# PRBonn/OverlapNet

Measured on AMD Instinct MI355X. Metric: scan-pairs/s (64x900 range images), higher is better.
Workload: dtype f32 (scaled 3-term fp16 split on the fp16 MFMA: 22 significand bits per operand, fp32 accumulate)

## Files before the change

overlapnet_amd/csrc/c3_dense.hip:

```cpp
#include "ovn_internal.h"

typedef _Float16 f16x8 __attribute__((ext_vector_type(8)));
typedef _Float16 f16x4 __attribute__((ext_vector_type(4)));

namespace {

struct ArithF16 {
  typedef _Float16 elem;
  typedef f16x8 v8;
  typedef f16x4 v4;
  static __device__ __forceinline__ f32x4 mfma(v8 a, v8 b, f32x4 c) { return __builtin_amdgcn_mfma_f32_16x16x32_f16(a, b, c, 0, 0, 0); }
};

constexpr int G = OVN_G;
constexpr int OW = OVN_O3_HW;
constexpr int CI = OVN_C2_OUT;
constexpr int CO = OVN_C3_OUT;
constexpr int NBAND = 3;
constexpr int MAX_ROWS = 8;
constexpr int MAX_MT = (MAX_ROWS * OW + 15) / 16;
constexpr int IN_PIX_MAX = (MAX_ROWS + 2) * G;
constexpr int PLANE = IN_PIX_MAX * 8 + 8;
constexpr int NPL = CI / 8;
constexpr size_t LDS_BYTES = 2 * (size_t)NPL * PLANE * sizeof(_Float16) + 64;
constexpr int NW = 8;

__device__ __forceinline__ int band_start(int b) { return b == 0 ? 0 : (b == 1 ? 8 : 15); }
__device__ __forceinline__ int band_rows(int b) { return b == 0 ? 8 : 7; }

constexpr int MT_SPLIT = 6;
template <class A, int NWV, int MSPLIT>
__global__ __launch_bounds__(64 * NWV) void c3_dense_kernel(const float* __restrict__ o2, const typename A::elem* __restrict__ wp,
                                                           const float* __restrict__ b3, const float* __restrict__ wd,
                                                           const unsigned* __restrict__ o2max, float sw3,
                                                           float* __restrict__ partial, float* __restrict__ o3,
                                                           unsigned* __restrict__ arrived, const float* __restrict__ bd,
                                                           float* __restrict__ overlap, float* __restrict__ logit) {
  typedef typename A::elem elem_t;
  typedef typename A::v8 v8_t;
  typedef typename A::v4 v4_t;
  extern __shared__ __attribute__((aligned(16))) unsigned char smem[];
  elem_t* ih = reinterpret_cast<elem_t*>(smem);
  elem_t* il = ih + NPL * PLANE;
  float* red = reinterpret_cast<float*>(il + NPL * PLANE);

  constexpr int HALVES = NW / NWV;
  constexpr int MTW = MSPLIT == 1 ? MAX_MT : MT_SPLIT;
  const int sub = blockIdx.x % (HALVES * MSPLIT);
  const int unit = blockIdx.x / (HALVES * MSPLIT), half = sub % HALVES, mh = sub / HALVES;
  const int mt0 = MT_SPLIT * mh;
  const int pair = unit / NBAND;
  const int band = unit - pair * NBAND;
  const int r0 = band_start(band);
  const int nrows = band_rows(band);
  const int npix = nrows * OW;
  const int nmt = (npix + 15) >> 4;
  const int tid = threadIdx.x;
  const int lane = tid & 63;
  const int wave_l = tid >> 6;
  const int wave = wave_l + NWV * half;
  const int lrow = lane & 15;
  const int g = lane >> 4;

  const elem_t* wsrc = wp + ((size_t)(2 * wave) * 2) * 512 + lane * 8;
  v8_t bq[3][4];
#define C3_LOAD_B(DST, KC)                                                                  \
  {                                                                                         \
    const elem_t* q = wsrc + (size_t)(KC) * (16 * 2 * 512);                                 \
    DST[0] = *reinterpret_cast<const v8_t*>(q);                                           \
    DST[1] = *reinterpret_cast<const v8_t*>(q + 512);                                     \
    DST[2] = *reinterpret_cast<const v8_t*>(q + 1024);                                    \
    DST[3] = *reinterpret_cast<const v8_t*>(q + 1536);                                    \
  }
  C3_LOAD_B(bq[0], 0)
  C3_LOAD_B(bq[1], 1)
  const float s2 = ovn_pow2_scale_for(__uint_as_float(o2max[pair]));
  const float inv = 1.0f / (s2 * sw3);
  {
    const float* src = o2 + ((long long)pair * G + r0) * G * CI;
    const int n4 = (nrows + 2) * G * CI / 4;
    constexpr int PER_THREAD = (MAX_ROWS + 2) * G * CI / 4 / (64 * NWV);
    static_assert(PER_THREAD * 64 * NWV == (MAX_ROWS + 2) * G * CI / 4, "patch does not divide over the threads");
    f32x4 v[PER_THREAD];
#pragma unroll
    for (int k = 0; k < PER_THREAD; ++k) {
      const int i = tid + k * (64 * NWV);
      v[k] = (i < n4) ? *reinterpret_cast<const f32x4*>(src + 4 * i) : (f32x4){0.f, 0.f, 0.f, 0.f};
    }
#pragma unroll
    for (int k = 0; k < PER_THREAD; ++k) {
      const int i = tid + k * (64 * NWV);
      if (i < n4) {
        const int pix = i / (CI / 4);
        const int c = 4 * (i - pix * (CI / 4));
        v4_t h, l;
#pragma unroll
        for (int e = 0; e < 4; ++e) {
          const float x = v[k][e] * s2;
          h[e] = (elem_t)x;
          l[e] = (elem_t)(x - (float)h[e]);
        }
        const int o = (c >> 3) * PLANE + pix * 8 + (c & 7);
        *reinterpret_cast<v4_t*>(ih + o) = h;
        *reinterpret_cast<v4_t*>(il + o) = l;
      }
    }
  }

  int abase[MTW];
#pragma unroll
  for (int mt = 0; mt < MTW; ++mt) {
    int p = 16 * (mt0 + mt) + lrow;
    if (p >= npix) p = npix - 1;
    const int oy = p / OW;
    const int ox = p - oy * OW;
    abase[mt] = g * PLANE + (oy * G + ox) * 8;
  }

  f32x4 acc[MTW][2];
#pragma unroll
  for (int mt = 0; mt < MTW; ++mt) {
    acc[mt][0] = (f32x4){0.f, 0.f, 0.f, 0.f};
    acc[mt][1] = (f32x4){0.f, 0.f, 0.f, 0.f};
  }

#define C3_MFMA2(M0, M1, A0H, A0L, A1H, A1L, SRC)                                                  \
  acc[M0][0] = A::mfma(A0H, SRC[0], acc[M0][0]);          \
  acc[M0][1] = A::mfma(A0H, SRC[2], acc[M0][1]);          \
  acc[M1][0] = A::mfma(A1H, SRC[0], acc[M1][0]);          \
  acc[M1][1] = A::mfma(A1H, SRC[2], acc[M1][1]);          \
  acc[M0][0] = A::mfma(A0L, SRC[0], acc[M0][0]);          \
  acc[M0][1] = A::mfma(A0L, SRC[2], acc[M0][1]);          \
  acc[M1][0] = A::mfma(A1L, SRC[0], acc[M1][0]);          \
  acc[M1][1] = A::mfma(A1L, SRC[2], acc[M1][1]);          \
  acc[M0][0] = A::mfma(A0H, SRC[1], acc[M0][0]);          \
  acc[M0][1] = A::mfma(A0H, SRC[3], acc[M0][1]);          \
  acc[M1][0] = A::mfma(A1H, SRC[1], acc[M1][0]);          \
  acc[M1][1] = A::mfma(A1H, SRC[3], acc[M1][1]);
#define C3_READ_A(BUF, SLOT, MT)                                                            \
  fh[BUF][SLOT] = *reinterpret_cast<const v8_t*>(ih + abase[MT] + toff);                  \
  fl[BUF][SLOT] = *reinterpret_cast<const v8_t*>(il + abase[MT] + toff);
#define C3_STEP(SRC, KC)                                                                    \
  {                                                                                         \
    const int tap = (KC) >> 2;                                                              \
    const int ky = tap / 3;                                                                 \
    const int toff = (ky * G + (tap - 3 * ky)) * 8 + 4 * PLANE * ((KC) & 3);                \
    v8_t fh[2][2], fl[2][2];                                                              \
    C3_READ_A(0, 0, 0)                                                                      \
    C3_READ_A(0, 1, 1)                                                                      \
    _Pragma("unroll") for (int q = 0; q < MTW / 2; ++q) {                                \
      const int cb = q & 1, nb = cb ^ 1;                                                    \
      if (q + 1 < MTW / 2) {                                                             \
        C3_READ_A(nb, 0, 2 * q + 2)                                                         \
        C3_READ_A(nb, 1, 2 * q + 3)                                                         \
      } else if (MTW % 2 == 1 && nmt == MAX_MT) {                                                           \
        C3_READ_A(nb, 0, MTW - 1)                                                        \
      }                                                                                     \
      __builtin_amdgcn_sched_barrier(0);   \
      C3_MFMA2(2 * q, 2 * q + 1, fh[cb][0], fl[cb][0], fh[cb][1], fl[cb][1], SRC)           \
      __builtin_amdgcn_sched_barrier(0);                                                    \
    }                                                                                       \
    if (MTW % 2 == 1 && nmt == MAX_MT) {                               \
      const v8_t ah = fh[(MTW / 2) & 1][0], al = fl[(MTW / 2) & 1][0];              \
      acc[MTW - 1][0] = A::mfma(ah, SRC[0], acc[MTW - 1][0]); \
      acc[MTW - 1][1] = A::mfma(ah, SRC[2], acc[MTW - 1][1]); \
      acc[MTW - 1][0] = A::mfma(al, SRC[0], acc[MTW - 1][0]); \
      acc[MTW - 1][1] = A::mfma(al, SRC[2], acc[MTW - 1][1]); \
      acc[MTW - 1][0] = A::mfma(ah, SRC[1], acc[MTW - 1][0]); \
      acc[MTW - 1][1] = A::mfma(ah, SRC[3], acc[MTW - 1][1]); \
    }                                                                                       \
  }
  __syncthreads();
#pragma unroll 1
  for (int kc = 0; kc < 36; kc += 3) {
    C3_LOAD_B(bq[2], kc + 2)
    C3_STEP(bq[0], kc)
    if (kc + 3 < 36) C3_LOAD_B(bq[0], kc + 3)
    C3_STEP(bq[1], kc + 1)
    if (kc + 4 < 36) C3_LOAD_B(bq[1], kc + 4)
    C3_STEP(bq[2], kc + 2)
  }
#undef C3_LOAD_B
#undef C3_STEP
#undef C3_MFMA2
#undef C3_READ_A

  float s[2] = {0.f, 0.f};
#pragma unroll
  for (int nt = 0; nt < 2; ++nt) {
    const int n = 32 * wave + 16 * nt + lrow;
    const float bv = b3[n];
#pragma unroll
    for (int mt = 0; mt < MTW; ++mt) {
#pragma unroll
      for (int r = 0; r < 4; ++r) {
        const int p = 16 * (mt0 + mt) + 4 * g + r;
        if (p < npix) {
          const float v = fmaxf(fmaf(acc[mt][nt][r], inv, bv), 0.0f);
          const long long fi = (long long)(r0 * OW + p) * CO + n;
          s[(MSPLIT == 1 && mt >= MT_SPLIT) ? 1 : 0] += v * wd[fi];
          if (o3) o3[(long long)pair * OVN_DENSE_IN + fi] = v;
        }
      }
    }
  }
#pragma unroll
  for (int off = 32; off > 0; off >>= 1) {
    s[0] += __shfl_down(s[0], off, 64);
    if (MSPLIT == 1) s[1] += __shfl_down(s[1], off, 64);
  }
  if (lane == 0) {
    red[wave_l] = s[0];
    if (MSPLIT == 1) red[NW + wave_l] = s[1];
  }
  __syncthreads();
  if (tid == 0) {
    float* dst = partial + ((size_t)pair * NBAND + band) * 4;
    if (NWV == NW) {
      dst[0] = (red[0] + red[1]) + (red[2] + red[3]);
      dst[1] = (red[NW + 0] + red[NW + 1]) + (red[NW + 2] + red[NW + 3]);
      dst[2] = (red[4] + red[5]) + (red[6] + red[7]);
      dst[3] = (red[NW + 4] + red[NW + 5]) + (red[NW + 6] + red[NW + 7]);
    } else {
      dst[2 * half + mh] = (red[0] + red[1]) + (red[2] + red[3]);
    }
    if (overlap != nullptr) {
      constexpr unsigned PARTS = NBAND * HALVES * MSPLIT;
      __threadfence();
      const unsigned prev = atomicAdd(arrived + pair, 1u);
      if (prev == PARTS - 1) {
        __threadfence();
        const float* q = partial + (size_t)pair * OVN_DENSE_PARTIALS;
        float z = 0.f;
#pragma unroll
        for (int b = 0; b < NBAND; ++b) {
          const float q0 = __hip_atomic_load(q + 4 * b, __ATOMIC_RELAXED, __HIP_MEMORY_SCOPE_AGENT);
          const float q1 = __hip_atomic_load(q + 4 * b + 1, __ATOMIC_RELAXED, __HIP_MEMORY_SCOPE_AGENT);
          const float q2 = __hip_atomic_load(q + 4 * b + 2, __ATOMIC_RELAXED, __HIP_MEMORY_SCOPE_AGENT);
          const float q3 = __hip_atomic_load(q + 4 * b + 3, __ATOMIC_RELAXED, __HIP_MEMORY_SCOPE_AGENT);
          const float zb = (q0 + q1) + (q2 + q3);
          z = b == 0 ? zb : z + zb;
        }
        z += bd[0];
        if (logit) logit[pair] = z;
        overlap[pair] = 1.0f / (1.0f + expf(-z));
        __hip_atomic_store(arrived + pair, 0u, __ATOMIC_RELAXED, __HIP_MEMORY_SCOPE_AGENT);
      }
    }
  }
}

__global__ __launch_bounds__(256) void dense_finish_kernel(const float* __restrict__ partial, const float* __restrict__ bd, int n,
                                                           float* __restrict__ overlap, float* __restrict__ logit) {
  const int p = blockIdx.x * 256 + threadIdx.x;
  if (p >= n) return;
  const float* q = partial + (size_t)p * OVN_DENSE_PARTIALS;
  float z = 0.f;
#pragma unroll
  for (int b = 0; b < NBAND; ++b) {
    const float zb = (q[4 * b] + q[4 * b + 1]) + (q[4 * b + 2] + q[4 * b + 3]);
    z = b == 0 ? zb : z + zb;
  }
  z += bd[0];
  if (logit) logit[p] = z;
  overlap[p] = 1.0f / (1.0f + expf(-z));
}

}

int ovn_c3_dense_forward(const ovn_ctx* ctx, const float* o2, const unsigned* o2max, int n, float* partial, float* o3,
                         unsigned* arrived, float* overlap, float* logit, hipStream_t stream) {
  OVN_REQUIRE(o2max != nullptr, OVN_ERR_ARG, "ovn_c3_dense_forward: the per-pair maxima of o2 are required");
  OVN_REQUIRE(overlap == nullptr || arrived != nullptr, OVN_ERR_ARG, "ovn_c3_dense_forward: arrival counters missing");
  int rc;
  if (n <= 21) {
    rc = ovn_allow_dynamic_lds(reinterpret_cast<const void*>(c3_dense_kernel<ArithF16, 4, 2>), LDS_BYTES);
    if (rc) return rc;
    hipLaunchKernelGGL((c3_dense_kernel<ArithF16, 4, 2>), dim3(4 * NBAND * n), dim3(64 * 4), LDS_BYTES, stream, o2,
                       reinterpret_cast<const _Float16*>(ctx->c3.wp_h), ctx->c3.bias, ctx->wd, o2max, ctx->c3.sw_h, partial, o3, arrived,
                       ctx->bd, overlap, logit);
  } else {
    rc = ovn_allow_dynamic_lds(reinterpret_cast<const void*>(c3_dense_kernel<ArithF16, NW, 1>), LDS_BYTES);
    if (rc) return rc;
    hipLaunchKernelGGL((c3_dense_kernel<ArithF16, NW, 1>), dim3(NBAND * n), dim3(64 * NW), LDS_BYTES, stream, o2,
                       reinterpret_cast<const _Float16*>(ctx->c3.wp_h), ctx->c3.bias, ctx->wd, o2max, ctx->c3.sw_h, partial, o3,
                       (unsigned*)nullptr, ctx->bd, (float*)nullptr, (float*)nullptr);
    if (overlap != nullptr)
      hipLaunchKernelGGL(dense_finish_kernel, dim3((n + 255) / 256), dim3(256), 0, stream, partial, ctx->bd, n, overlap, logit);
  }
  OVN_HIP_CHECK(hipGetLastError());
  return OVN_OK;
}
```

overlapnet_amd/csrc/ovn_api.hip:

```cpp
#include <stdarg.h>
#include <mutex>
#include <set>
#include <utility>
#include <stdio.h>
#include <stdlib.h>
#include <string.h>

#include <algorithm>
#include "ovn_internal.h"

int ovn_allow_dynamic_lds(const void* kernel, size_t bytes) {
  static std::mutex mu;
  static std::set<std::pair<const void*, int>> done;
  int dev = 0;
  OVN_HIP_CHECK(hipGetDevice(&dev));
  std::lock_guard<std::mutex> lock(mu);
  if (done.count({kernel, dev})) return OVN_OK;
  OVN_HIP_CHECK(hipFuncSetAttribute(kernel, hipFuncAttributeMaxDynamicSharedMemorySize, (int)bytes));
  done.insert({kernel, dev});
  return OVN_OK;
}

static thread_local char g_err[1024] = "";

void ovn_set_error(const char* fmt, ...) {
  va_list ap;
  va_start(ap, fmt);
  vsnprintf(g_err, sizeof(g_err), fmt, ap);
  va_end(ap);
}

void scratch_overwritten(ovn_ctx* ctx) {
  ctx->dbg_o2 = ctx->dbg_o3 = nullptr;
  ctx->dbg_partial = nullptr;
  ctx->dbg_o2max = nullptr;
  ctx->dbg_n = 0;
  ctx->dbg_live = nullptr;
}

int ovn_ws_reserve(ovn_ctx* ctx, size_t bytes, hipStream_t stream) {
  if (bytes <= ctx->ws_bytes) return OVN_OK;
  if (ctx->ws) {
    OVN_HIP_CHECK(hipStreamSynchronize(stream));
    OVN_HIP_CHECK(hipFree(ctx->ws));
    ctx->ws = nullptr;
    ctx->ws_bytes = 0;
    scratch_overwritten(ctx);
  }
  const size_t want = bytes + bytes / 8;
  OVN_HIP_CHECK(hipMalloc(&ctx->ws, want));
  ctx->ws_bytes = want;
  return OVN_OK;
}

static int ctx_feat_w(const ovn_ctx* ctx) { return ctx->finalized ? ctx->feat_w : OVN_FEAT_W; }

struct LegScratch {
  float* buf[2] = {nullptr, nullptr};
  double *acc = nullptr, *part = nullptr;
  LegScratch() = default;
  LegScratch(OvnCarver& c, size_t buf_elems, int nbuf, size_t acc_elems, size_t part_bytes) {
    for (int i = 0; i < nbuf; ++i) buf[i] = c.take<float>(buf_elems);
    acc = c.take<double>(acc_elems);
    part = reinterpret_cast<double*>(c.take<char>(part_bytes));
  }
};

extern "C" {

int ovn_abi_version(void) { return OVN_ABI_VERSION; }

const char* ovn_last_error(void) { return g_err; }

int ovn_create(int device_id, int in_h, int in_w, int in_c, ovn_ctx** out) {
  OVN_REQUIRE(out != nullptr, OVN_ERR_ARG, "ovn_create: out is NULL");
  OVN_REQUIRE(in_h > 0 && in_w > 0 && in_c > 0, OVN_ERR_ARG, "ovn_create: bad input shape %dx%dx%d", in_h, in_w, in_c);
  int ndev = 0;
  OVN_HIP_CHECK(hipGetDeviceCount(&ndev));
  OVN_REQUIRE(device_id >= 0 && device_id < ndev, OVN_ERR_ARG, "ovn_create: device %d not present (%d devices)", device_id, ndev);
  OVN_ON_DEVICE(device_id);
  hipDeviceProp_t prop;
  OVN_HIP_CHECK(hipGetDeviceProperties(&prop, device_id));
  OVN_REQUIRE(strncmp(prop.gcnArchName, "gfx950", 6) == 0, OVN_ERR_STATE,
              "ovn_create: this library is built for gfx950 only, device %d is %s", device_id, prop.gcnArchName);
  ovn_ctx* c = new ovn_ctx();
  c->device = device_id;
  c->in_h = in_h;
  c->in_w = in_w;
  c->in_c = in_c;
  if (const char* e = getenv("OVN_HEAD_CHUNK")) c->head_chunk = atoll(e) > 0 ? atoll(e) : c->head_chunk;
  if (const char* e = getenv("OVN_HEAD_SUBCHUNK")) c->head_sub = atoll(e) >= 0 ? atoll(e) : c->head_sub;
  if (const char* e = getenv("OVN_HEAD_STREAMS")) c->head_streams = atoi(e) == 2 ? 2 : 1;
  if (const char* e = getenv("OVN_YAW_SIDE")) c->head_yaw_side = atoi(e) ? 1 : 0;
  int rc = ovn_spectral_prepare(c, nullptr);
  if (rc) {
    ovn_conv_release(&c->dft);
    if (c->tw64) (void)hipFree(c->tw64);
    delete c;
    return rc;
  }
  *out = c;
  return OVN_OK;
}

int ovn_destroy(ovn_ctx* ctx) {
  if (!ctx) return OVN_OK;
  if (ctx->comm) (void)ovn_comm_destroy(ctx);
  OVN_ON_DEVICE(ctx->device);
  (void)hipDeviceSynchronize();
  for (auto& l : ctx->leg) ovn_conv_release(&l);
  ovn_conv_release(&ctx->c2);
  ovn_conv_release(&ctx->c3);
  ovn_conv_release(&ctx->dft);
  if (ctx->tw64) (void)hipFree(ctx->tw64);
  if (ctx->w1p) (void)hipFree(ctx->w1p);
  if (ctx->b1) (void)hipFree(ctx->b1);
  if (ctx->wd) (void)hipFree(ctx->wd);
  if (ctx->bd) (void)hipFree(ctx->bd);
  if (ctx->w1p_h) (void)hipFree(ctx->w1p_h);
  if (ctx->w2p_h) (void)hipFree(ctx->w2p_h);
  if (ctx->w1raw) (void)hipFree(ctx->w1raw);
  if (ctx->w1sum) (void)hipFree(ctx->w1sum);
  if (ctx->w1col) (void)hipFree(ctx->w1col);
  if (ctx->wsp_h) (void)hipFree(ctx->wsp_h);
  if (ctx->w2sum) (void)hipFree(ctx->w2sum);
  if (ctx->w1p_b3) (void)hipFree(ctx->w1p_b3);
  if (ctx->w2p_b3) (void)hipFree(ctx->w2p_b3);
  if (ctx->w2raw) (void)hipFree(ctx->w2raw);
  if (ctx->w3raw) (void)hipFree(ctx->w3raw);
  if (ctx->ws) (void)hipFree(ctx->ws);
  if (ctx->norm_buf) (void)hipFree(ctx->norm_buf);
  if (ctx->actmax) (void)hipFree(ctx->actmax);
  if (ctx->c3_arrived) (void)hipFree(ctx->c3_arrived);
  if (ctx->seg_dev) (void)hipFree(ctx->seg_dev);
  if (ctx->seg_host) (void)hipHostFree(ctx->seg_host);
  if (ctx->seg_ev) (void)hipEventDestroy(ctx->seg_ev);
  if (ctx->seg_done) (void)hipEventDestroy(ctx->seg_done);
  if (ctx->aux_ready) {
    for (int i = 0; i < 2; ++i) {
      (void)hipStreamDestroy(ctx->aux[i]);
      (void)hipEventDestroy(ctx->ev_join[i]);
    }
    (void)hipEventDestroy(ctx->ev_fork);
  }
  delete ctx;
  return OVN_OK;
}

static int leg_layer_prepare(OvnConvLayer* L, const float* kernel_dev, const float* bias_dev, hipStream_t stream) {
  int rc = ovn_conv_prepare(L, kernel_dev, bias_dev, stream);
  if (rc == OVN_OK) rc = ovn_conv_prepare_f16x3(L, kernel_dev, stream);
  if (rc == OVN_OK) {
    const size_t bytes = (size_t)L->kh * L->kw * L->cin * L->cout * sizeof(float);
    hipError_t e = hipMalloc((void**)&L->wraw, bytes);
    if (e == hipSuccess) e = hipMemcpyAsync(L->wraw, kernel_dev, bytes, hipMemcpyDeviceToDevice, stream);
    if (e == hipSuccess) e = hipStreamSynchronize(stream);
    if (e != hipSuccess) {
      ovn_set_error("layer %s: keeping the raw kernel failed: %s", L->name.c_str(), hipGetErrorString(e));
      rc = OVN_ERR_HIP;
    }
  }
  if (rc) ovn_conv_release(L);
  return rc;
}

int ovn_add_leg_layer(ovn_ctx* ctx, const char* name, const float* kernel_dev, const float* bias_dev, int kh, int kw,
                      int cin, int cout, int stride_h, int stride_w, void* stream) {
  OVN_REQUIRE(ctx && name && kernel_dev && bias_dev, OVN_ERR_ARG, "ovn_add_leg_layer: NULL argument");
  OVN_REQUIRE(kh > 0 && kw > 0 && cin > 0 && cout > 0 && stride_h > 0 && stride_w > 0, OVN_ERR_ARG,
              "ovn_add_leg_layer(%s): bad geometry", name);
  OVN_REQUIRE(!ctx->finalized, OVN_ERR_STATE, "ovn_add_leg_layer(%s): context already finalized", name);
  const int expect_cin = ctx->leg.empty() ? ctx->in_c : ctx->leg.back().cout;
  OVN_REQUIRE(cin == expect_cin, OVN_ERR_ARG, "ovn_add_leg_layer(%s): cin=%d but previous layer produces %d", name, cin, expect_cin);
  OVN_ON_DEVICE(ctx->device);
  OvnConvLayer L;
  L.name = name;
  L.kh = kh;
  L.kw = kw;
  L.cin = cin;
  L.cout = cout;
  L.sh = stride_h;
  L.sw = stride_w;
  L.relu = 1;
  int rc = leg_layer_prepare(&L, kernel_dev, bias_dev, (hipStream_t)stream);
  if (rc) return rc;
  ctx->leg.push_back(L);
  return OVN_OK;
}

int ovn_set_leg_layer_weights(ovn_ctx* ctx, int layer, const float* kernel_dev, const float* bias_dev, void* stream) {
  OVN_REQUIRE(ctx && kernel_dev && bias_dev, OVN_ERR_ARG, "ovn_set_leg_layer_weights: NULL argument");
  OVN_REQUIRE(ctx->finalized, OVN_ERR_STATE, "ovn_set_leg_layer_weights: context not finalized");
  OVN_REQUIRE(layer >= 0 && layer < (int)ctx->leg.size(), OVN_ERR_ARG, "ovn_set_leg_layer_weights: no such leg layer %d", layer);
  OVN_ON_DEVICE(ctx->device);
  OvnConvLayer N = ctx->leg[layer];
  N.wp = N.bias = N.wraw = nullptr;
  N.wp_h = N.wp_h16 = nullptr;
  N.sw_h = 1.f;
  int rc = leg_layer_prepare(&N, kernel_dev, bias_dev, (hipStream_t)stream);
  if (rc) return rc;
  ovn_conv_release(&ctx->leg[layer]);
  ctx->leg[layer] = N;
  return OVN_OK;
}

int ovn_set_head_weights(ovn_ctx* ctx, const float* c1k, const float* c1b, const float* c2k, const float* c2b,
                         const float* c3k, const float* c3b, const float* dk, const float* db, void* stream_) {
  OVN_REQUIRE(ctx && c1k && c1b && c2k && c2b && c3k && c3b && dk && db, OVN_ERR_ARG, "ovn_set_head_weights: NULL argument");
  OVN_ON_DEVICE(ctx->device);
  hipStream_t stream = (hipStream_t)stream_;
  {
    ovn_conv_release(&ctx->c2);
    ovn_conv_release(&ctx->c3);
    if (ctx->w1p) (void)hipFree(ctx->w1p);
    if (ctx->b1) (void)hipFree(ctx->b1);
    if (ctx->wd) (void)hipFree(ctx->wd);
    if (ctx->bd) (void)hipFree(ctx->bd);
    if (ctx->w1p_h) (void)hipFree(ctx->w1p_h);
    if (ctx->w2p_h) (void)hipFree(ctx->w2p_h);
    if (ctx->w1raw) (void)hipFree(ctx->w1raw);
    if (ctx->w1sum) (void)hipFree(ctx->w1sum);
    if (ctx->w1col) (void)hipFree(ctx->w1col);
    if (ctx->wsp_h) (void)hipFree(ctx->wsp_h);
      if (ctx->w2sum) (void)hipFree(ctx->w2sum);
    if (ctx->w1p_b3) (void)hipFree(ctx->w1p_b3);
    if (ctx->w2p_b3) (void)hipFree(ctx->w2p_b3);
    if (ctx->w2raw) (void)hipFree(ctx->w2raw);
    if (ctx->w3raw) (void)hipFree(ctx->w3raw);
    ctx->w3raw = nullptr;
    ctx->w1p_h = ctx->w2p_h = ctx->wsp_h = ctx->w1p_b3 = ctx->w2p_b3 = nullptr;
    ctx->w1raw = ctx->w1sum = ctx->w1col = ctx->w2sum = ctx->w2raw = nullptr;
    ctx->w1p = ctx->b1 = ctx->wd = ctx->bd = nullptr;
    ctx->head_set = false;
  }
  ctx->head_g = ctx_feat_w(ctx) / ctx->head_s;
  const int hs = ctx->head_s, hg = ctx->head_g;
  OVN_REQUIRE(hg >= 3, OVN_ERR_ARG, "ovn_set_head_weights: conv1size %d leaves %d column groups, c_conv3 needs 3", hs, hg);
  const bool general = (hs != OVN_S);
  int rc = OVN_OK;
  if (!general) {
    rc = ovn_delta_prepare_w1(c1k, &ctx->w1p, stream);
    if (rc) return rc;
  } else {
    const size_t w1_bytes = (size_t)hs * OVN_FEAT_C * OVN_C1_OUT * sizeof(float);
    OVN_HIP_CHECK(hipMalloc((void**)&ctx->w1raw, w1_bytes));
    OVN_HIP_CHECK(hipMemcpyAsync(ctx->w1raw, c1k, w1_bytes, hipMemcpyDeviceToDevice, stream));
  }
  OVN_HIP_CHECK(hipMalloc((void**)&ctx->b1, OVN_C1_OUT * sizeof(float)));
  OVN_HIP_CHECK(hipMemcpyAsync(ctx->b1, c1b, OVN_C1_OUT * sizeof(float), hipMemcpyDeviceToDevice, stream));
  ctx->c2 = OvnConvLayer();
  ctx->c2.name = "c_conv2";
  ctx->c2.kh = hs;
  ctx->c2.kw = 1;
  ctx->c2.cin = OVN_C1_OUT;
  ctx->c2.cout = OVN_C2_OUT;
  ctx->c2.sh = hs;
  ctx->c2.sw = 1;
  ctx->c2.relu = 1;
  rc = ovn_conv_prepare(&ctx->c2, c2k, c2b, stream);
  if (rc) return rc;
  if (!general) {
    rc = ovn_delta_prepare_f16x3(ctx, c1k, c1b, c2k, stream);
    if (rc) return rc;
  }
  ctx->c3 = OvnConvLayer();
  ctx->c3.name = "c_conv3";
  ctx->c3.kh = 3;
  ctx->c3.kw = 3;
  ctx->c3.cin = OVN_C2_OUT;
  ctx->c3.cout = OVN_C3_OUT;
  ctx->c3.sh = 1;
  ctx->c3.sw = 1;
  ctx->c3.relu = 1;
  rc = ovn_conv_prepare(&ctx->c3, c3k, c3b, stream);
  if (rc) return rc;
  if (!general) {
    rc = ovn_conv_prepare_f16x3(&ctx->c3, c3k, stream);
    if (rc) return rc;
  }
  const size_t w3_bytes = (size_t)9 * OVN_C2_OUT * OVN_C3_OUT * sizeof(float);
  OVN_HIP_CHECK(hipMalloc((void**)&ctx->w3raw, w3_bytes));
  OVN_HIP_CHECK(hipMemcpyAsync(ctx->w3raw, c3k, w3_bytes, hipMemcpyDeviceToDevice, stream));
  if (!ctx->w2raw) {
    const size_t w2_bytes = (size_t)hs * OVN_C1_OUT * OVN_C2_OUT * sizeof(float);
    OVN_HIP_CHECK(hipMalloc((void**)&ctx->w2raw, w2_bytes));
    OVN_HIP_CHECK(hipMemcpyAsync(ctx->w2raw, c2k, w2_bytes, hipMemcpyDeviceToDevice, stream));
  }
  const size_t dense_in = (size_t)(hg - 2) * (hg - 2) * OVN_C3_OUT;
  OVN_HIP_CHECK(hipMalloc((void**)&ctx->wd, dense_in * sizeof(float)));
  OVN_HIP_CHECK(hipMalloc((void**)&ctx->bd, sizeof(float)));
  OVN_HIP_CHECK(hipMemcpyAsync(ctx->wd, dk, dense_in * sizeof(float), hipMemcpyDeviceToDevice, stream));
  OVN_HIP_CHECK(hipMemcpyAsync(ctx->bd, db, sizeof(float), hipMemcpyDeviceToDevice, stream));
  OVN_HIP_CHECK(hipStreamSynchronize(stream));
  ctx->head_set = true;
  return OVN_OK;
}

static int leg_f16x3_unserved(const ovn_ctx* ctx) {
  int h = ctx->in_h, w = ctx->in_w;
  for (size_t li = 0; li < ctx->leg.size(); ++li) {
    const auto& l = ctx->leg[li];
    if (h < l.kh || w < l.kw) return -1;
    const int oh = (h - l.kh) / l.sh + 1, ow = (w - l.kw) / l.sw + 1;
    if (li == 0 && ovn_leg_front_matches(ctx, li, h, w)) {
      const auto& l2 = ctx->leg[1];
      h = (oh - l2.kh) / l2.sh + 1;
      w = (ow - l2.kw) / l2.sw + 1;
      ++li;
      continue;
    }
    if (ovn_leg_tail_matches(ctx, li, h, w)) return -1;
    if (!ovn_conv_strip_matches(l, h, w) && (long long)oh * ow < 128) return (int)li;
    h = oh;
    w = ow;
  }
  return -1;
}

int ovn_finalize(ovn_ctx* ctx, int* feat_w) {
  OVN_REQUIRE(ctx != nullptr, OVN_ERR_ARG, "ovn_finalize: ctx is NULL");
  OVN_REQUIRE(!ctx->leg.empty(), OVN_ERR_STATE, "ovn_finalize: no leg layers registered");
  int h = ctx->in_h, w = ctx->in_w, c = ctx->in_c;
  for (const auto& l : ctx->leg) {
    OVN_REQUIRE(h >= l.kh && w >= l.kw, OVN_ERR_ARG, "ovn_finalize: layer %s does not fit its %dx%d input", l.name.c_str(), h, w);
    h = (h - l.kh) / l.sh + 1;
    w = (w - l.kw) / l.sw + 1;
    c = l.cout;
  }
  OVN_REQUIRE(h == 1 && w >= OVN_FEAT_W_MIN && w <= OVN_FEAT_W_MAX && c == OVN_FEAT_C, OVN_ERR_ARG,
              "ovn_finalize: leg produces %dx%dx%d, the heads need 1 x W x %d with %d <= W <= %d", h, w, c, OVN_FEAT_C, OVN_FEAT_W_MIN,
              OVN_FEAT_W_MAX);
  OVN_REQUIRE(!ctx->head_set || w / ctx->head_s == ctx->head_g, OVN_ERR_STATE,
              "ovn_finalize: leg width %d gives %d column groups, the head weights were registered for %d", w, w / ctx->head_s,
              ctx->head_g);
  if (ctx->leg_mode != 0) {
    const int bad = leg_f16x3_unserved(ctx);
    OVN_REQUIRE(bad < 0, OVN_ERR_ARG,
                "ovn_finalize: layer %s: fewer than 128 output positions per image in leg precision f16x3 (ovn_set_leg_precision(ctx, 0) "
                "before ovn_finalize runs this leg in fp32)", ctx->leg[bad < 0 ? 0 : bad].name.c_str());
  }
  ctx->feat_w = w;
  ctx->finalized = true;
  if (feat_w) *feat_w = w;
  return OVN_OK;
}

int ovn_leg(ovn_ctx* ctx, const float* images_dev, int64_t n, float* features_dev, void* stream_) {
  OVN_REQUIRE(ctx && ctx->finalized, OVN_ERR_STATE, "ovn_leg: context not finalized");
  OVN_REQUIRE(n >= 0, OVN_ERR_ARG, "ovn_leg: n < 0");
  if (n == 0) return OVN_OK;
  OVN_REQUIRE(images_dev && features_dev, OVN_ERR_ARG, "ovn_leg: NULL buffer");
  OVN_ON_DEVICE(ctx->device);
  hipStream_t stream = (hipStream_t)stream_;
  size_t max_act = 0;
  {
    int h = ctx->in_h, w = ctx->in_w;
    for (const auto& l : ctx->leg) {
      h = (h - l.kh) / l.sh + 1;
      w = (w - l.kw) / l.sw + 1;
      const size_t e = (size_t)h * w * l.cout;
      if (e > max_act) max_act = e;
    }
  }
  const int64_t nslices = (n + OVN_LEG_SLICE - 1) / OVN_LEG_SLICE;
  const int64_t slice = (n + nslices - 1) / nslices;
  LegScratch sc;
  int rc = ovn_ws_layout(ctx, stream, &sc, (size_t)slice * max_act, 2, (size_t)0, (size_t)0);
  if (rc) return rc;
  float* const* buf = sc.buf;
  const size_t in_elems = (size_t)ctx->in_h * ctx->in_w * ctx->in_c;
  const size_t feat_elems = (size_t)ctx->feat_w * OVN_FEAT_C;
  OVN_REQUIRE(ctx->leg.size() + 1 <= OVN_ACTMAX_SLOTS, OVN_ERR_STATE, "ovn_leg: too many leg layers");
  const size_t actmax_bytes = (size_t)OVN_ACTMAX_SLOTS * OVN_LEG_SLICE * OVN_ACTMAX_STRIDE * sizeof(unsigned);
  if (ctx->leg_mode != 0 && !ctx->actmax) OVN_HIP_CHECK(hipMalloc((void**)&ctx->actmax, actmax_bytes));
  for (int64_t s0 = 0; s0 < n; s0 += slice) {
    const int nb = (int)((n - s0 < slice) ? (n - s0) : slice);
    const float* cur = images_dev + (size_t)s0 * in_elems;
    int h = ctx->in_h, w = ctx->in_w;
    if (ctx->leg_mode != 0) {
      OVN_HIP_CHECK(hipMemsetAsync(ctx->actmax, 0, (ctx->leg.size() + 1) * (size_t)slice * OVN_ACTMAX_STRIDE * sizeof(unsigned), stream));
      const bool own = (reinterpret_cast<uintptr_t>(cur) & 15) == 0 && ovn_conv_strip_own_scale(ctx->leg[0], h, w);
      if (!own) {
        OvnProfScope ps(ctx, OVN_K_LEG, stream);
        rc = ovn_absmax_forward(cur, nb, (long long)in_elems, ctx->actmax, stream);
        if (rc) return rc;
      }
    }
    for (size_t li = 0; li < ctx->leg.size(); ++li) {
      const bool last = (li + 1 == ctx->leg.size());
      float* dst = last ? features_dev + (size_t)s0 * feat_elems : buf[li & 1];
      int oh = 0, ow = 0;
      if (ctx->leg_mode != 0 && li == 0 && (reinterpret_cast<uintptr_t>(cur) & 15) == 0 && ovn_leg_front_matches(ctx, li, h, w)) {
        OvnProfScope ps(ctx, OVN_K_LEG, stream);
        float* dst2 = buf[(li + 1) & 1];
        rc = ovn_leg_front_forward(ctx, li, cur, nb, h, w, dst2, &oh, &ow, ctx->actmax + (li + 2) * (size_t)slice * OVN_ACTMAX_STRIDE, stream);
        if (rc) return rc;
        cur = dst2;
        h = oh;
        w = ow;
        ++li;
        continue;
      }
      if (ctx->leg_mode != 0 && ovn_leg_tail_matches(ctx, li, h, w)) {
        OvnProfScope ps(ctx, OVN_K_LEG, stream);
        rc = ovn_leg_tail_forward(ctx, li, cur, nb, w, features_dev + (size_t)s0 * feat_elems, stream);
        if (rc) return rc;
        break;
      }
      {
        OvnProfScope ps(ctx, OVN_K_LEG, stream);
        rc = (ctx->leg_mode == 0) ? ovn_conv_forward(ctx->leg[li], cur, nb, h, w, dst, &oh, &ow, stream)
                                  : ovn_conv_forward_f16x3(ctx->leg[li], cur, nb, h, w, dst, &oh, &ow, ctx->actmax + li * (size_t)slice * OVN_ACTMAX_STRIDE,
                                                           last ? nullptr : ctx->actmax + (li + 1) * (size_t)slice * OVN_ACTMAX_STRIDE, stream);
      }
      if (rc) return rc;
      cur = dst;
      h = oh;
      w = ow;
    }
  }
  return OVN_OK;
}

struct LegGeom {
  std::vector<int> h, w;
  std::vector<int64_t> act;
  int64_t act_total = 0, act_max = 0, params = 0;
};

static LegGeom leg_geom(const ovn_ctx* ctx) {
  LegGeom g;
  int h = ctx->in_h, w = ctx->in_w;
  for (const auto& l : ctx->leg) {
    g.h.push_back(h);
    g.w.push_back(w);
    h = (h - l.kh) / l.sh + 1;
    w = (w - l.kw) / l.sw + 1;
    g.act.push_back((int64_t)h * w * l.cout);
    g.act_total += g.act.back();
    g.act_max = std::max(g.act_max, g.act.back());
    g.params += (int64_t)l.kh * l.kw * l.cin * l.cout + l.cout;
  }
  return g;
}

int ovn_leg_layer_count(ovn_ctx* ctx, int* layers) {
  OVN_REQUIRE(ctx && layers, OVN_ERR_ARG, "ovn_leg_layer_count: NULL argument");
  *layers = (int)ctx->leg.size();
  return OVN_OK;
}

int ovn_leg_param_sizes(ovn_ctx* ctx, int64_t* sizes) {
  OVN_REQUIRE(ctx && sizes, OVN_ERR_ARG, "ovn_leg_param_sizes: NULL argument");
  for (size_t li = 0; li < ctx->leg.size(); ++li) {
    const auto& l = ctx->leg[li];
    sizes[2 * li] = (int64_t)l.kh * l.kw * l.cin * l.cout;
    sizes[2 * li + 1] = l.cout;
  }
  return OVN_OK;
}

int ovn_leg_activation_sizes(ovn_ctx* ctx, int64_t* sizes) {
  OVN_REQUIRE(ctx && sizes, OVN_ERR_ARG, "ovn_leg_activation_sizes: NULL argument");
  OVN_REQUIRE(ctx->finalized, OVN_ERR_STATE, "ovn_leg_activation_sizes: context not finalized");
  const LegGeom g = leg_geom(ctx);
  for (size_t li = 0; li < g.act.size(); ++li) sizes[li] = g.act[li];
  return OVN_OK;
}

int ovn_leg_forward_train(ovn_ctx* ctx, const float* images_dev, int64_t n, float* acts_dev, void* stream_) {
  OVN_REQUIRE(ctx && images_dev && acts_dev, OVN_ERR_ARG, "ovn_leg_forward_train: NULL argument");
  OVN_REQUIRE(n >= 1 && n < (1ll << 31), OVN_ERR_ARG, "ovn_leg_forward_train: bad n %lld", (long long)n);
  OVN_REQUIRE(ctx->finalized, OVN_ERR_STATE, "ovn_leg_forward_train: context not finalized");
  OVN_ON_DEVICE(ctx->device);
  hipStream_t stream = (hipStream_t)stream_;
  const LegGeom g = leg_geom(ctx);
  const float* cur = images_dev;
  float* dst = acts_dev;
  for (size_t li = 0; li < ctx->leg.size(); ++li) {
    OvnProfScope ps(ctx, OVN_K_LEG, stream);
    int oh = 0, ow = 0;
    int rc = ovn_conv_forward(ctx->leg[li], cur, (int)n, g.h[li], g.w[li], dst, &oh, &ow, stream);
    if (rc) return rc;
    cur = dst;
    dst += (size_t)n * g.act[li];
  }
  return OVN_OK;
}

int ovn_leg_backward(ovn_ctx* ctx, const float* images_dev, const float* acts_dev, int64_t n, const float* dfeat_dev, float* grad_dev,
                     int64_t slice_scans, void* stream_) {
  OVN_REQUIRE(ctx && images_dev && acts_dev && dfeat_dev && grad_dev, OVN_ERR_ARG, "ovn_leg_backward: NULL argument");
  OVN_REQUIRE(n >= 1 && n < (1ll << 31), OVN_ERR_ARG, "ovn_leg_backward: bad n %lld", (long long)n);
  OVN_REQUIRE(slice_scans >= 0, OVN_ERR_ARG, "ovn_leg_backward: slice_scans %lld < 0", (long long)slice_scans);
  OVN_REQUIRE(ctx->finalized, OVN_ERR_STATE, "ovn_leg_backward: context not finalized");
  OVN_ON_DEVICE(ctx->device);
  hipStream_t stream = (hipStream_t)stream_;
  const LegGeom g = leg_geom(ctx);
  const int L = (int)ctx->leg.size();
  constexpr int64_t SB = OVN_LEG_GRAD_SCAN_BLOCK;
  int64_t slice = slice_scans == 0 ? 8 * SB : std::max<int64_t>(SB, slice_scans / SB * SB);
  slice = std::min(slice, std::min<int64_t>((n + SB - 1) / SB * SB, 65535 / SB * SB));
  const int nmax = (int)std::min(slice, n);
  size_t part_bytes = 0;
  for (int li = 0; li < L; ++li) part_bytes = std::max(part_bytes, ovn_leg_grad_part_bytes(ctx->leg[li], g.h[li], g.w[li], nmax));
  LegScratch sc;
  int rc = ovn_ws_layout(ctx, stream, &sc, (size_t)nmax * g.act_max, 2, (size_t)g.params, part_bytes);
  if (rc) return rc;
  scratch_overwritten(ctx);
  float* const* buf = sc.buf;
  double *acc = sc.acc, *part = sc.part;
  OVN_HIP_CHECK(hipMemsetAsync(acc, 0, (size_t)g.params * sizeof(double), stream));
  std::vector<int64_t> act_off(L, 0), par_off(L, 0);
  for (int li = 1; li < L; ++li) {
    act_off[li] = act_off[li - 1] + g.act[li - 1];
    par_off[li] = par_off[li - 1] + (int64_t)ctx->leg[li - 1].K * ctx->leg[li - 1].cout + ctx->leg[li - 1].cout;
  }
  const size_t in_elems = (size_t)ctx->in_h * ctx->in_w * ctx->in_c;
  for (int64_t s0 = 0; s0 < n; s0 += slice) {
    const int nb = (int)std::min(slice, n - s0);
    OvnProfScope ps(ctx, OVN_K_LEG, stream);
    int cur = 0;
    rc = ovn_leg_mask_forward(dfeat_dev + (size_t)s0 * g.act[L - 1], acts_dev + (size_t)n * act_off[L - 1] + (size_t)s0 * g.act[L - 1],
                              buf[cur], (long long)nb * g.act[L - 1], stream);
    if (rc) return rc;
    for (int li = L - 1; li >= 0; --li) {
      const auto& l = ctx->leg[li];
      const float* x = li ? acts_dev + (size_t)n * act_off[li - 1] + (size_t)s0 * g.act[li - 1] : images_dev + (size_t)s0 * in_elems;
      double* ak = acc + par_off[li];
      rc = ovn_leg_layer_backward(l, x, buf[cur], nb, g.h[li], g.w[li], li ? buf[cur ^ 1] : nullptr, li ? x : nullptr, ak,
                                  ak + (int64_t)l.K * l.cout, part, stream);
      if (rc) return rc;
      cur ^= 1;
    }
  }
  return ovn_leg_grad_round(acc, grad_dev, g.params, stream);
}

int ovn_debug_conv_grad(ovn_ctx* ctx, int layer, const float* in_dev, const float* out_dev, const float* dout_dev, int nb, int h, int w,
                        float* din_dev, float* dkernel_dev, float* dbias_dev, void* stream_) {
  OVN_REQUIRE(ctx && in_dev && out_dev && dout_dev, OVN_ERR_ARG, "ovn_debug_conv_grad: NULL argument");
  OVN_REQUIRE(layer >= 0 && layer < (int)ctx->leg.size(), OVN_ERR_ARG, "ovn_debug_conv_grad: no such leg layer %d", layer);
  OVN_REQUIRE(nb >= 1 && nb <= 65535, OVN_ERR_ARG, "ovn_debug_conv_grad: bad nb %d", nb);
  const OvnConvLayer& l = ctx->leg[layer];
  OVN_REQUIRE(h >= l.kh && w >= l.kw, OVN_ERR_ARG, "ovn_debug_conv_grad: input %dx%d smaller than the kernel of %s", h, w, l.name.c_str());
  OVN_ON_DEVICE(ctx->device);
  hipStream_t stream = (hipStream_t)stream_;
  const int oh = (h - l.kh) / l.sh + 1, ow = (w - l.kw) / l.sw + 1;
  const long long out_elems = (long long)nb * oh * ow * l.cout;
  const int64_t kelems = (int64_t)l.K * l.cout;
  LegScratch sc;
  int rc = ovn_ws_layout(ctx, stream, &sc, (size_t)out_elems, 1, (size_t)(kelems + l.cout), ovn_leg_grad_part_bytes(l, h, w, nb));
  if (rc) return rc;
  scratch_overwritten(ctx);
  float* dym = sc.buf[0];
  double *acc = sc.acc, *part = sc.part;
  OVN_HIP_CHECK(hipMemsetAsync(acc, 0, (size_t)(kelems + l.cout) * sizeof(double), stream));
  OvnProfScope ps(ctx, OVN_K_LEG, stream);
  rc = ovn_leg_mask_forward(dout_dev, out_dev, dym, out_elems, stream);
  if (rc) return rc;
  rc = ovn_leg_layer_backward(l, in_dev, dym, nb, h, w, din_dev, nullptr, dkernel_dev ? acc : nullptr, dbias_dev ? acc + kelems : nullptr,
                              part, stream);
  if (rc) return rc;
  if (dkernel_dev) rc = ovn_leg_grad_round(acc, dkernel_dev, kelems, stream);
  if (rc == OVN_OK && dbias_dev) rc = ovn_leg_grad_round(acc + kelems, dbias_dev, l.cout, stream);
  return rc;
}

int ovn_corr_head(ovn_ctx* ctx, const float* feats_l, const int32_t* lidx, const float* feats_r, const int32_t* ridx,
                  int64_t n, int32_t* yaw, float* corr, void* stream) {
  OVN_REQUIRE(ctx != nullptr, OVN_ERR_ARG, "ovn_corr_head: ctx is NULL");
  OVN_REQUIRE(n >= 0 && n < (1ll << 31), OVN_ERR_ARG, "ovn_corr_head: bad n");
  if (n == 0) return OVN_OK;
  OVN_REQUIRE(feats_l && feats_r && yaw, OVN_ERR_ARG, "ovn_corr_head: NULL buffer");
  OVN_ON_DEVICE(ctx->device);
  OvnProfScope ps(ctx, OVN_K_CORR, (hipStream_t)stream);
  return ovn_corr_forward(feats_l, lidx, feats_r, ridx, (int)n, ctx_feat_w(ctx), yaw, corr, (hipStream_t)stream, ctx->corr_norm);
}

int ovn_spectrum(ovn_ctx* ctx, const float* feats_dev, int64_t n, float* spectra_dev, void* stream) {
  OVN_REQUIRE(ctx != nullptr, OVN_ERR_ARG, "ovn_spectrum: ctx is NULL");
  OVN_REQUIRE(ctx_feat_w(ctx) == OVN_FEAT_W, OVN_ERR_ARG,
              "ovn_spectrum: the spectral correlation head needs 360-column feature volumes (the leg produces %d)", ctx_feat_w(ctx));
  OVN_REQUIRE(n >= 0 && n < (1ll << 24), OVN_ERR_ARG, "ovn_spectrum: bad n");
  if (n == 0) return OVN_OK;
  OVN_REQUIRE(feats_dev && spectra_dev, OVN_ERR_ARG, "ovn_spectrum: NULL buffer");
  OVN_ON_DEVICE(ctx->device);
  OvnProfScope ps(ctx, OVN_K_SPECTRUM, (hipStream_t)stream);
  return ovn_spectrum_forward(ctx, feats_dev, (int)n, spectra_dev, (hipStream_t)stream);
}

int ovn_corr_head_spectral(ovn_ctx* ctx, const float* spec_l, const int32_t* lidx, const float* spec_r,
                           const int32_t* ridx, int64_t n, int32_t* yaw, float* corr, void* stream) {
  OVN_REQUIRE(ctx != nullptr, OVN_ERR_ARG, "ovn_corr_head_spectral: ctx is NULL");
  OVN_REQUIRE(ctx_feat_w(ctx) == OVN_FEAT_W, OVN_ERR_ARG,
              "ovn_corr_head_spectral: the spectral correlation head needs 360-column feature volumes (the leg produces %d)", ctx_feat_w(ctx));
  OVN_REQUIRE(n >= 0 && n < (1ll << 31), OVN_ERR_ARG, "ovn_corr_head_spectral: bad n");
  if (n == 0) return OVN_OK;
  OVN_REQUIRE(spec_l && spec_r && yaw, OVN_ERR_ARG, "ovn_corr_head_spectral: NULL buffer");
  OVN_ON_DEVICE(ctx->device);
  OvnProfScope ps(ctx, OVN_K_CORR_SPECTRAL, (hipStream_t)stream);
  return ovn_corr_spectral_forward(ctx, spec_l, lidx, spec_r, ridx, (int)n, yaw, corr, (hipStream_t)stream);
}

static int head_streams_ready(ovn_ctx* ctx) {
  if (ctx->aux_ready) return OVN_OK;
  for (int i = 0; i < 2; ++i) {
    OVN_HIP_CHECK(hipStreamCreateWithFlags(&ctx->aux[i], hipStreamNonBlocking));
    OVN_HIP_CHECK(hipEventCreateWithFlags(&ctx->ev_join[i], hipEventDisableTiming));
  }
  OVN_HIP_CHECK(hipEventCreateWithFlags(&ctx->ev_fork, hipEventDisableTiming));
  ctx->aux_ready = true;
  return OVN_OK;
}

struct OvnFork {
  ovn_ctx* ctx;
  hipStream_t stream;
  bool used[2] = {false, false};
  bool forked = false;
  OvnFork(ovn_ctx* c, hipStream_t s) : ctx(c), stream(s) {}
  int fork() {
    if (forked) return OVN_OK;
    int rc = head_streams_ready(ctx);
    if (rc) return rc;
    OVN_HIP_CHECK(hipEventRecord(ctx->ev_fork, stream));
    forked = true;
    return OVN_OK;
  }
  int side(int i, hipStream_t* out) {
    int rc = fork();
    if (rc) return rc;
    if (!used[i]) {
      OVN_HIP_CHECK(hipStreamWaitEvent(ctx->aux[i], ctx->ev_fork, 0));
      used[i] = true;
    }
    *out = ctx->aux[i];
    return OVN_OK;
  }
  int join() {
    int rc = OVN_OK;
    for (int i = 0; i < 2; ++i)
      if (used[i]) {
        used[i] = false;
        if (hipEventRecord(ctx->ev_join[i], ctx->aux[i]) != hipSuccess || hipStreamWaitEvent(stream, ctx->ev_join[i], 0) != hipSuccess) {
          ovn_set_error("joining the head's side stream failed");
          rc = OVN_ERR_HIP;
        }
      }
    return rc;
  }
  ~OvnFork() { (void)join(); }
};

static int delta_head_run_f32(ovn_ctx* ctx, const float* feats_l, const int32_t* lidx, const float* feats_r, const int32_t* ridx,
                              int64_t n, float* overlap, float* logit, int32_t* yaw, float* corr, int corr_mode, const float* spec_l,
                              const float* spec_r, hipStream_t stream) {
  const int fw = ctx_feat_w(ctx);
  const size_t feat_elems = (size_t)fw * OVN_FEAT_C;
  OVN_REQUIRE(corr_mode != 2 || fw == OVN_FEAT_W, OVN_ERR_ARG, "spectral correlation head at feature width %d", fw);
  const bool fusedc12 = (ctx->head_s == OVN_S);
  const size_t pb = fusedc12 ? ovn_delta_pair_bytes(ctx->head_g) : ovn_delta_generic_pair_bytes(fw, ctx->head_g);
  int64_t chunk = (int64_t)((2ull << 30) / pb);
  chunk = chunk < 1 ? 1 : (chunk > 1024 ? 1024 : chunk);
  if (ctx->head_chunk < chunk) chunk = ctx->head_chunk;
  const int64_t cmax = n < chunk ? n : chunk;
  OvnDeltaF32Scratch sc;
  OvnDeltaGenericScratch gsc;
  int rc = fusedc12 ? ovn_ws_layout(ctx, stream, &sc, cmax, ctx->head_g, ctx->head_width_split && ctx->head_mode == 1)
                    : ovn_ws_layout(ctx, stream, &gsc, cmax, fw, ctx->head_g);
  if (rc) return rc;
  scratch_overwritten(ctx);
  OvnFork fk(ctx, stream);
  if (corr_mode == 2) {
    hipStream_t ys = stream;
    if (ctx->head_yaw_side) {
      rc = fk.side(1, &ys);
      if (rc) return rc;
    }
    OvnProfScope ps(ctx, OVN_K_CORR_SPECTRAL, ys);
    rc = ovn_corr_spectral_forward(ctx, spec_l, lidx, spec_r, ridx, (int)n, yaw, corr, ys);
    if (rc) return rc;
  }
  for (int64_t p0 = 0; p0 < n; p0 += chunk) {
    const int np = (int)((n - p0 < chunk) ? (n - p0) : chunk);
    const float* fl = lidx ? feats_l : feats_l + (size_t)p0 * feat_elems;
    const int32_t* li = lidx ? lidx + p0 : nullptr;
    const int32_t* ri = ridx ? ridx + p0 : nullptr;
    if (corr_mode == 1) {
      OvnProfScope ps(ctx, OVN_K_CORR, stream);
      rc = ovn_corr_forward(fl, li, feats_r, ri, np, fw, yaw + p0, corr ? corr + (size_t)p0 * fw : nullptr, stream, ctx->corr_norm);
      if (rc) return rc;
    }
    if (fusedc12) {
      rc = ovn_delta_forward(ctx, fl, li, feats_r, ri, np, sc, overlap + p0, logit ? logit + p0 : nullptr, stream);
    } else {
      OvnProfScope ps(ctx, OVN_K_DELTA, stream);
      rc = ovn_delta_generic_forward(ctx, fl, li, feats_r, ri, np, gsc, overlap + p0, logit ? logit + p0 : nullptr, stream);
    }
    if (rc) return rc;
  }
  if (fusedc12 && n > 0 && n <= chunk) {
    ctx->dbg_o2 = sc.o2;
    ctx->dbg_o3 = sc.o3;
    ctx->dbg_n = n;
  }
  return fk.join();
}

struct HeadScratch {
  float *o2 = nullptr, *o3 = nullptr;
  char* sub = nullptr;
  size_t sub_bytes = 0;
  OvnDeltaSegScratch seg;
  HeadScratch() = default;
  HeadScratch(OvnCarver& c, int64_t cmax, bool fused, int64_t sub_pairs, int nsub, bool per_pair_right, int nseg) {
    o2 = c.take<float>((size_t)cmax * OVN_G * OVN_G * OVN_C2_OUT);
    o3 = c.take<float>((size_t)cmax * (fused ? OVN_DENSE_PARTIALS : OVN_DENSE_IN));
    sub_bytes = ovn_delta_f16x3_scratch_bytes((int)sub_pairs, per_pair_right);
    sub = c.take<char>(sub_bytes * nsub);
    if (nseg) seg = OvnDeltaSegScratch(c, nseg);
  }
  OvnDeltaSubScratch sub_chunk(int j, int np, bool per_pair_right) const {
    OvnCarver c(sub + (size_t)j * sub_bytes);
    return OvnDeltaSubScratch(c, np, per_pair_right);
  }
};

static int delta_head_run(ovn_ctx* ctx, const float* feats_l, const int32_t* lidx, const float* feats_r,
                          const int32_t* ridx, int64_t n, float* overlap, float* logit, int32_t* yaw, float* corr,
                          int corr_mode, const float* spec_l, const float* spec_r, const float* dcache_l, hipStream_t stream,
                          const OvnSegPass* seg = nullptr) {
  ctx->dbg_live = nullptr;
  const int fw = ctx_feat_w(ctx);
  if (ctx->head_s != OVN_S || fw != OVN_FEAT_W || ctx->head_mode == 0)
    return delta_head_run_f32(ctx, feats_l, lidx, feats_r, ridx, n, overlap, logit, yaw, corr, corr_mode, spec_l, spec_r, stream);
  const size_t feat_elems = (size_t)fw * OVN_FEAT_C;
  const size_t o2_elems = (size_t)OVN_G * OVN_G * OVN_C2_OUT;
  const size_t o3_elems = (size_t)OVN_DENSE_IN;
  const bool fused = (ctx->head_mode == 1);
  const int64_t chunk = ctx->head_chunk;
  const int64_t cmax = n < chunk ? n : chunk;
  int64_t sub = (!seg && ctx->head_sub > 0 && ctx->head_sub < cmax) ? ctx->head_sub : cmax;
  const int nsub_max = (int)((cmax + sub - 1) / sub);
  const int nstreams = (nsub_max > 1 && ctx->head_streams > 1) ? 2 : 1;
  HeadScratch hs;
  int rc = ovn_ws_layout(ctx, stream, &hs, cmax, fused, sub, nsub_max, ridx != nullptr, seg ? seg->nseg : 0);
  if (rc) return rc;
  if (fused && ctx->c3_arrived_n < chunk) {
    OVN_HIP_CHECK(hipStreamSynchronize(stream));
    if (ctx->c3_arrived) (void)hipFree(ctx->c3_arrived);
    ctx->c3_arrived = nullptr;
    ctx->c3_arrived_n = 0;
    OVN_HIP_CHECK(hipMalloc((void**)&ctx->c3_arrived, (size_t)chunk * sizeof(unsigned)));
    OVN_HIP_CHECK(hipMemsetAsync(ctx->c3_arrived, 0, (size_t)chunk * sizeof(unsigned), stream));
    ctx->c3_arrived_n = chunk;
  }
  float *o2 = hs.o2, *o3 = hs.o3;
  ctx->dbg_o2max = nullptr;
  ctx->dbg_o2 = o2;
  ctx->dbg_o3 = fused ? nullptr : o3;
  ctx->dbg_partial = fused ? o3 : nullptr;
  ctx->dbg_n = sub < cmax ? sub : cmax;

  OvnFork fk(ctx, stream);
  bool a2_in_yaw = false;
  if (corr_mode == 2) {
    hipStream_t ys = stream;
    if (ctx->head_yaw_side) {
      rc = fk.side(1, &ys);
      if (rc) return rc;
    }
    OvnProfScope ps(ctx, OVN_K_CORR_SPECTRAL, ys);
    a2_in_yaw = ridx == nullptr && n <= OVN_A2_IN_YAW_MAX_PAIRS && n <= chunk && ys == stream && nsub_max == 1;
    rc = ovn_corr_spectral_forward(ctx, spec_l, lidx, spec_r, ridx, (int)n, yaw, corr, ys, a2_in_yaw ? feats_r : nullptr,
                                   a2_in_yaw ? hs.sub_chunk(0, (int)n, false).a2raw : nullptr);
    if (rc) return rc;
  }
  for (int64_t c0 = 0; c0 < n; c0 += chunk) {
    const int64_t cn = (n - c0 < chunk) ? (n - c0) : chunk;
    if (corr_mode == 1) {
      OvnProfScope ps(ctx, OVN_K_CORR, stream);
      rc = ovn_corr_forward(lidx ? feats_l : feats_l + (size_t)c0 * feat_elems, lidx ? lidx + c0 : nullptr, feats_r,
                            ridx ? ridx + c0 : nullptr, (int)cn, fw, yaw + c0, corr ? corr + (size_t)c0 * fw : nullptr, stream,
                            ctx->corr_norm);
      if (rc) return rc;
    }
    int j = 0;
    for (int64_t q0 = 0; q0 < cn; q0 += sub, ++j) {
      const int64_t p0 = c0 + q0;
      const int np = (int)((cn - q0 < sub) ? (cn - q0) : sub);
      hipStream_t st = stream;
      if (nstreams == 2 && (j & 1)) {
        rc = fk.side(0, &st);
        if (rc) return rc;
      }
      const float* fl = lidx ? feats_l : feats_l + (size_t)p0 * feat_elems;
      const int32_t* li = lidx ? lidx + p0 : nullptr;
      const int32_t* ri = ridx ? ridx + p0 : nullptr;
      float* o2s = o2 + (size_t)q0 * o2_elems;
      const OvnDeltaSubScratch ds = hs.sub_chunk(j, np, ridx != nullptr);
      if (fused) {
        unsigned* o2max = ds.o2max;
        float* part = o3 + (size_t)q0 * OVN_DENSE_PARTIALS;
        OvnSegPass sp{};
        if (seg) {
          sp = *seg;
          sp.pseg += p0;
          sp.state = hs.seg;
        }
        rc = ovn_delta_c12_f16x3_forward(ctx, fl, li, feats_r, ri, np, ds, o2s, st, (int)(p0 & 0x3fffffff),
                                          dcache_l ? (lidx ? dcache_l : dcache_l + (size_t)p0 * OVN_DELTA_CACHE_ELEMS) : nullptr, a2_in_yaw,
                                          seg ? &sp : nullptr);
        if (rc) return rc;
        if (p0 == 0) ctx->dbg_o2max = o2max;
        {
          OvnProfScope ps(ctx, OVN_K_C3, st);
          rc = ovn_c3_dense_forward(ctx, o2s, o2max, np, part, nullptr, ctx->c3_arrived + q0, overlap + p0, logit ? logit + p0 : nullptr, st);
        }
      } else {
        float* o3s = o3 + (size_t)q0 * o3_elems;
        rc = ovn_delta_c12_bf16x3_forward(ctx, fl, li, feats_r, ri, np, ds, o2s, st, (int)(p0 & 0x3fffffff),
                                          a2_in_yaw);
        if (rc) return rc;
        int oh = 0, ow = 0;
        {
          OvnProfScope ps(ctx, OVN_K_C3, st);
          rc = ovn_conv_forward(ctx->c3, o2s, np, OVN_G, OVN_G, o3s, &oh, &ow, st);
        }
        if (rc) return rc;
        OvnProfScope ps(ctx, OVN_K_DENSE, st);
        rc = ovn_dense_sigmoid_forward(ctx, o3s, np, OVN_DENSE_IN, overlap + p0, logit ? logit + p0 : nullptr, st);
      }
      if (rc) return rc;
    }
  }
  return fk.join();
}

int ovn_heads(ovn_ctx* ctx, const float* feats_l, const int32_t* lidx, const float* feats_r, const int32_t* ridx,
              int64_t n, float* overlap, int32_t* yaw, float* logit, float* corr, void* stream_) {
  OVN_REQUIRE(ctx && ctx->head_set, OVN_ERR_STATE, "ovn_heads: head weights not set");
  OVN_REQUIRE(n >= 0 && n < (1ll << 31), OVN_ERR_ARG, "ovn_heads: bad n");
  if (n == 0) return OVN_OK;
  OVN_REQUIRE(feats_l && feats_r && overlap && yaw, OVN_ERR_ARG, "ovn_heads: NULL buffer");
  OVN_ON_DEVICE(ctx->device);
  return delta_head_run(ctx, feats_l, lidx, feats_r, ridx, n, overlap, logit, yaw, corr, 1, nullptr, nullptr, nullptr, (hipStream_t)stream_);
}

int ovn_heads_spectral(ovn_ctx* ctx, const float* feats_l, const float* spec_l, const float* dcache_l, const int32_t* lidx,
                       const float* feats_r, const float* spec_r, const int32_t* ridx, int64_t n, float* overlap, int32_t* yaw,
                       float* logit, float* corr, void* stream_) {
  OVN_REQUIRE(ctx && ctx->head_set, OVN_ERR_STATE, "ovn_heads_spectral: head weights not set");
  OVN_REQUIRE(ctx_feat_w(ctx) == OVN_FEAT_W, OVN_ERR_ARG,
              "ovn_heads_spectral: the spectral correlation head needs 360-column feature volumes (the leg produces %d)", ctx_feat_w(ctx));
  OVN_REQUIRE(n >= 0 && n < (1ll << 31), OVN_ERR_ARG, "ovn_heads_spectral: bad n");
  if (n == 0) return OVN_OK;
  OVN_REQUIRE(feats_l && feats_r && spec_l && spec_r && overlap && yaw, OVN_ERR_ARG, "ovn_heads_spectral: NULL buffer");
  OVN_ON_DEVICE(ctx->device);
  return delta_head_run(ctx, feats_l, lidx, feats_r, ridx, n, overlap, logit, yaw, corr, 2, spec_l, spec_r,
                        ctx->head_mode == 1 ? dcache_l : nullptr, (hipStream_t)stream_);
}

int ovn_delta_head(ovn_ctx* ctx, const float* feats_l, const int32_t* lidx, const float* feats_r, const int32_t* ridx,
                   int64_t n, float* overlap, float* logit, void* stream_) {
  OVN_REQUIRE(ctx && ctx->head_set, OVN_ERR_STATE, "ovn_delta_head: head weights not set");
  OVN_REQUIRE(n >= 0 && n < (1ll << 31), OVN_ERR_ARG, "ovn_delta_head: bad n");
  if (n == 0) return OVN_OK;
  OVN_REQUIRE(feats_l && feats_r && overlap, OVN_ERR_ARG, "ovn_delta_head: NULL buffer");
  OVN_ON_DEVICE(ctx->device);
  return delta_head_run(ctx, feats_l, lidx, feats_r, ridx, n, overlap, logit, nullptr, nullptr, 0, nullptr, nullptr, nullptr, (hipStream_t)stream_);
}

int ovn_head_param_sizes(ovn_ctx* ctx, int64_t* sizes8) {
  OVN_REQUIRE(ctx && sizes8, OVN_ERR_ARG, "ovn_head_param_sizes: NULL argument");
  ovn_head_param_sizes_of(ctx->head_s, ctx_feat_w(ctx), sizes8);
  return OVN_OK;
}

int ovn_delta_head_grad(ovn_ctx* ctx, const float* feats_l, const int32_t* lidx, const float* feats_r, const int32_t* ridx, int64_t n,
                        const float* target, int loss, float scale, float* grad, float* loss_dev, float* overlap, float* o2, float* o3,
                        void* stream_) {
  OVN_REQUIRE(ctx && feats_l && feats_r && target && grad && loss_dev, OVN_ERR_ARG, "ovn_delta_head_grad: NULL argument");
  OVN_REQUIRE(n >= 1 && n < (1ll << 31), OVN_ERR_ARG, "ovn_delta_head_grad: bad n %lld", (long long)n);
  OVN_REQUIRE(loss == 0 || loss == 1, OVN_ERR_ARG, "ovn_delta_head_grad: loss %d (0 = sigmoid loss, 1 = squared error)", loss);
  OVN_REQUIRE(isfinite(scale), OVN_ERR_ARG, "ovn_delta_head_grad: scale is not finite");
  OVN_REQUIRE(ctx->head_set, OVN_ERR_STATE, "ovn_delta_head_grad: head weights not set");
  OVN_ON_DEVICE(ctx->device);
  return ovn_delta_head_grad_run(ctx, ctx_feat_w(ctx), feats_l, lidx, feats_r, ridx, n, target, loss, scale, grad, loss_dev, overlap, o2,
                                 o3, (hipStream_t)stream_);
}

int ovn_heads_feature_grad(ovn_ctx* ctx, const float* feats_l, const int32_t* lidx, const float* feats_r, const int32_t* ridx, int64_t n,
                           const float* target, const int32_t* yaw_bin, int loss, float overlap_scale, float yaw_scale,
                           float min_overlap_for_angle, float* dfeat_l, float* dfeat_r, float* head_grad, float* loss_dev, float* overlap,
                           float* corr, void* stream_) {
  OVN_REQUIRE(ctx && feats_l && feats_r && target && dfeat_l && dfeat_r && loss_dev, OVN_ERR_ARG, "ovn_heads_feature_grad: NULL argument");
  OVN_REQUIRE(n >= 1 && n < (1ll << 31), OVN_ERR_ARG, "ovn_heads_feature_grad: bad n %lld", (long long)n);
  OVN_REQUIRE(loss == 0 || loss == 1, OVN_ERR_ARG, "ovn_heads_feature_grad: loss %d (0 = sigmoid loss, 1 = squared error)", loss);
  OVN_REQUIRE(isfinite(overlap_scale) && isfinite(yaw_scale) && isfinite(min_overlap_for_angle), OVN_ERR_ARG,
              "ovn_heads_feature_grad: a scale or the threshold is not finite");
  OVN_REQUIRE(ctx->head_set, OVN_ERR_STATE, "ovn_heads_feature_grad: head weights not set");
  const bool yaw_on = yaw_bin != nullptr && yaw_scale != 0.f;
  OVN_REQUIRE(!yaw_on || ctx->corr_norm == 0, OVN_ERR_STATE,
              "ovn_heads_feature_grad: the yaw loss is differentiated for correlation normalisation 'none' only (mode %d is set)",
              ctx->corr_norm);
  OVN_ON_DEVICE(ctx->device);
  hipStream_t stream = (hipStream_t)stream_;
  const int fw = ctx_feat_w(ctx);
  const size_t bytes = (size_t)n * fw * OVN_FEAT_C * sizeof(float);
  OVN_HIP_CHECK(hipMemsetAsync(dfeat_l, 0, bytes, stream));
  OVN_HIP_CHECK(hipMemsetAsync(dfeat_r, 0, bytes, stream));
  OVN_HIP_CHECK(hipMemsetAsync(loss_dev, 0, 2 * sizeof(float), stream));
  int rc = OVN_OK;
  if (overlap_scale != 0.f) {
    rc = ovn_delta_head_grad_run(ctx, fw, feats_l, lidx, feats_r, ridx, n, target, loss, overlap_scale, head_grad, loss_dev, overlap, nullptr,
                                 nullptr, stream, dfeat_l, dfeat_r);
  } else {
    if (head_grad) {
      int64_t sz[8], total = 0;
      ovn_head_param_sizes_of(ctx->head_s, fw, sz);
      for (int t = 0; t < 8; ++t) total += sz[t];
      OVN_HIP_CHECK(hipMemsetAsync(head_grad, 0, (size_t)total * sizeof(float), stream));
    }
    if (overlap)
      rc = ovn_delta_head_grad_run(ctx, fw, feats_l, lidx, feats_r, ridx, n, target, loss, 0.f, nullptr, nullptr, overlap, nullptr, nullptr,
                                   stream, nullptr, nullptr, true);
  }
  if (rc) return rc;
  if (yaw_on || corr)
    rc = ovn_yaw_grad_run(ctx, fw, feats_l, lidx, feats_r, ridx, n, target, yaw_on ? yaw_bin : nullptr, yaw_scale, min_overlap_for_angle,
                          dfeat_l, dfeat_r, loss_dev + 1, corr, stream);
  return rc;
}

int ovn_delta_cache(ovn_ctx* ctx, const float* feats_dev, int64_t n, float* cache_dev, void* stream) {
  OVN_REQUIRE(ctx && ctx->head_set, OVN_ERR_STATE, "ovn_delta_cache: head weights not set");
  OVN_REQUIRE(ctx_feat_w(ctx) == OVN_FEAT_W, OVN_ERR_ARG,
              "ovn_delta_cache: Delta cache rows exist for 360-column feature volumes only (the leg produces %d)", ctx_feat_w(ctx));
  OVN_REQUIRE(n >= 0 && n < (1ll << 24), OVN_ERR_ARG, "ovn_delta_cache: bad n");
  if (n == 0) return OVN_OK;
  OVN_REQUIRE(feats_dev && cache_dev, OVN_ERR_ARG, "ovn_delta_cache: NULL buffer");
  OVN_REQUIRE((reinterpret_cast<uintptr_t>(cache_dev) & 15) == 0, OVN_ERR_ARG, "ovn_delta_cache: cache_dev must be 16-byte aligned");
  OVN_REQUIRE(ctx->head_s == OVN_S, OVN_ERR_STATE, "ovn_delta_cache: only the default head geometry (conv1size 15) has a Delta cache");
  OVN_ON_DEVICE(ctx->device);
  OvnProfScope ps(ctx, OVN_K_DELTA_PREP, (hipStream_t)stream);
  return ovn_delta_cache_forward(ctx, feats_dev, (int)n, cache_dev, (hipStream_t)stream);
}

int ovn_set_head_geometry(ovn_ctx* ctx, int conv1size) {
  OVN_REQUIRE(ctx != nullptr, OVN_ERR_ARG, "ovn_set_head_geometry: ctx is NULL");
  OVN_REQUIRE(!ctx->head_set, OVN_ERR_STATE, "ovn_set_head_geometry: call it before ovn_set_head_weights");
  const int fw = ctx_feat_w(ctx);
  OVN_REQUIRE(conv1size >= 1 && fw / conv1size >= 3, OVN_ERR_ARG,
              "ovn_set_head_geometry: conv1size %d leaves fewer than 3 x 3 groups of the %d columns for c_conv3", conv1size, fw);
  ctx->head_s = conv1size;
  ctx->head_g = fw / conv1size;
  return OVN_OK;
}

int ovn_set_head_pipeline(ovn_ctx* ctx, int64_t chunk_pairs, int64_t sub_chunk_pairs, int streams, int yaw_on_side_stream) {
  OVN_REQUIRE(ctx != nullptr, OVN_ERR_ARG, "ovn_set_head_pipeline: ctx is NULL");
  OVN_REQUIRE(chunk_pairs >= 1 && chunk_pairs <= (1 << 20), OVN_ERR_ARG, "ovn_set_head_pipeline: chunk_pairs %lld", (long long)chunk_pairs);
  OVN_REQUIRE(sub_chunk_pairs >= 0, OVN_ERR_ARG, "ovn_set_head_pipeline: sub_chunk_pairs %lld", (long long)sub_chunk_pairs);
  OVN_REQUIRE(streams == 1 || streams == 2, OVN_ERR_ARG, "ovn_set_head_pipeline: streams %d (1 or 2)", streams);
  ctx->head_chunk = chunk_pairs;
  ctx->head_sub = sub_chunk_pairs;
  ctx->head_streams = streams;
  ctx->head_yaw_side = yaw_on_side_stream ? 1 : 0;
  return OVN_OK;
}

int ovn_get_head_pipeline(ovn_ctx* ctx, int64_t* chunk_pairs, int64_t* sub_chunk_pairs, int* streams, int* yaw_on_side_stream) {
  OVN_REQUIRE(ctx != nullptr, OVN_ERR_ARG, "ovn_get_head_pipeline: ctx is NULL");
  if (chunk_pairs) *chunk_pairs = ctx->head_chunk;
  if (sub_chunk_pairs) *sub_chunk_pairs = ctx->head_sub;
  if (streams) *streams = ctx->head_streams;
  if (yaw_on_side_stream) *yaw_on_side_stream = ctx->head_yaw_side;
  return OVN_OK;
}

int ovn_best_match(ovn_ctx* ctx, const float* overlap, const int32_t* yaw, const int32_t* ids, int64_t n, float threshold,
                   int64_t index_offset, int32_t* out, void* stream) {
  OVN_REQUIRE(ctx != nullptr, OVN_ERR_ARG, "ovn_best_match: ctx is NULL");
  OVN_REQUIRE(n >= 0 && n < (1ll << 31), OVN_ERR_ARG, "ovn_best_match: bad n");
  OVN_REQUIRE(index_offset >= 0 && index_offset + n < (1ll << 31), OVN_ERR_ARG, "ovn_best_match: bad index_offset");
  OVN_REQUIRE(out != nullptr && (n == 0 || overlap != nullptr), OVN_ERR_ARG, "ovn_best_match: NULL buffer");
  OVN_ON_DEVICE(ctx->device);
  return ovn_best_match_forward(overlap, yaw, ids, (int)n, threshold, (int)index_offset, out, (hipStream_t)stream);
}

int ovn_top_k(ovn_ctx* ctx, const float* overlap, const int32_t* yaw, const int32_t* ids, int64_t n, int k, float threshold,
              int64_t index_offset, int32_t* out, void* stream) {
  OVN_REQUIRE(ctx != nullptr, OVN_ERR_ARG, "ovn_top_k: ctx is NULL");
  OVN_REQUIRE(k >= 1 && k <= OVN_TOP_K_MAX, OVN_ERR_ARG, "ovn_top_k: k must be in 1..OVN_TOP_K_MAX (1024)");
  OVN_REQUIRE(n >= 0 && n < (1ll << 31), OVN_ERR_ARG, "ovn_top_k: bad n");
  OVN_REQUIRE(index_offset >= 0 && index_offset + n < (1ll << 31), OVN_ERR_ARG, "ovn_top_k: bad index_offset");
  OVN_REQUIRE(out != nullptr && (n == 0 || overlap != nullptr), OVN_ERR_ARG, "ovn_top_k: NULL buffer");
  OVN_REQUIRE((reinterpret_cast<uintptr_t>(out) & 15) == 0, OVN_ERR_ARG, "ovn_top_k: out_dev is not 16-byte aligned");
  OVN_ON_DEVICE(ctx->device);
  return ovn_top_k_forward(overlap, yaw, ids, (int)n, k, threshold, (int)index_offset, out, (hipStream_t)stream);
}

int ovn_icp_register(ovn_ctx* ctx, const float* vertex, const float* normal, const float* range, int n_scans, int proj_h, int proj_w,
                     double fov_up_deg, double fov_down_deg, double max_range, const int32_t* src_idx, const int32_t* tgt_idx,
                     int64_t n_pairs, const double* init_pose, int iterations, double max_dist, double cos_min, double huber,
                     int min_inliers, double* pose, double* stats, double* system, void* stream) {
  OVN_REQUIRE(ctx != nullptr, OVN_ERR_ARG, "ovn_icp_register: ctx is NULL");
  OVN_REQUIRE(n_scans >= 0 && proj_h > 0 && proj_w > 0 && n_pairs >= 0 && n_pairs < (1ll << 31), OVN_ERR_ARG,
              "ovn_icp_register: bad sizes");
  OVN_REQUIRE((int64_t)proj_h * proj_w <= 2147483647ll, OVN_ERR_ARG, "ovn_icp_register: H*W exceeds 2^31 - 1");
  OVN_REQUIRE(iterations >= 0 && iterations <= 1000, OVN_ERR_ARG, "ovn_icp_register: iterations must be in 0..1000");
  OVN_REQUIRE(max_dist > 0.0 && cos_min > 0.0 && huber > 0.0 && max_range > 0.0, OVN_ERR_ARG,
              "ovn_icp_register: max_dist, cos_min, huber and max_range must be > 0");
  OVN_REQUIRE(max_dist < 1e18 && cos_min <= 1.0 && huber < 1e18, OVN_ERR_ARG, "ovn_icp_register: gate out of range");
  OVN_REQUIRE(min_inliers >= 0, OVN_ERR_ARG, "ovn_icp_register: min_inliers < 0");
  OVN_REQUIRE(fabs(fov_up_deg) + fabs(fov_down_deg) > 0.0, OVN_ERR_ARG, "ovn_icp_register: empty vertical field of view");
  if (n_pairs == 0) return OVN_OK;
  OVN_REQUIRE(src_idx && tgt_idx && init_pose && pose && stats, OVN_ERR_ARG, "ovn_icp_register: NULL buffer");
  OVN_REQUIRE(n_scans == 0 || (vertex && normal && range), OVN_ERR_ARG, "ovn_icp_register: NULL image buffer");
  OVN_ON_DEVICE(ctx->device);
  return ovn_icp_register_forward(vertex, normal, range, n_scans, proj_h, proj_w, fov_up_deg, fov_down_deg, max_range, src_idx,
                                  tgt_idx, (int)n_pairs, init_pose, iterations, max_dist, cos_min, huber, min_inliers, pose, stats,
                                  system, (hipStream_t)stream);
}

struct SegTable {
  int64_t* offs = nullptr;
  int32_t *qidx = nullptr, *ridx = nullptr, *pseg = nullptr;
  SegTable() = default;
  SegTable(OvnCarver& c, int64_t B, bool with_qidx, int64_t n_ridx, int64_t n_pseg) {
    offs = c.take<int64_t>((size_t)B + 1);
    qidx = with_qidx ? c.take<int32_t>((size_t)B) : nullptr;
    ridx = n_ridx ? c.take<int32_t>((size_t)n_ridx) : nullptr;
    pseg = n_pseg ? c.take<int32_t>((size_t)n_pseg) : nullptr;
  }
};
static const char* seg_offsets_error(const int64_t* offs, int64_t B, int64_t* n_out) {
  if (B < 0 || B >= (1ll << 31)) return "B outside [0, 2^31)";
  if (!offs) return "seg_offsets is NULL";
  if (offs[0] != 0) return "seg_offsets[0] != 0";
  for (int64_t b = 0; b < B; ++b)
    if (offs[b + 1] < offs[b]) return "seg_offsets decrease";
  if (offs[B] >= (1ll << 31)) return "more than 2^31 - 1 pairs";
  *n_out = offs[B];
  return nullptr;
}

static int seg_stage(ovn_ctx* ctx, const int64_t* offs, const int32_t* qidx, int64_t B, int64_t n_ridx, int64_t n_pseg,
                     hipStream_t stream, SegTable* dev) {
  const size_t staged = ovn_scratch_bytes<SegTable>(B, qidx != nullptr, (int64_t)0, (int64_t)0);
  const size_t need = ovn_scratch_bytes<SegTable>(B, qidx != nullptr, n_ridx, n_pseg);
  if (!ctx->seg_ev) {
    OVN_HIP_CHECK(hipEventCreateWithFlags(&ctx->seg_ev, hipEventDisableTiming));
    OVN_HIP_CHECK(hipEventCreateWithFlags(&ctx->seg_done, hipEventDisableTiming));
  }
  if (ctx->seg_ev_pending) {
    OVN_HIP_CHECK(hipEventSynchronize(ctx->seg_ev));
    OVN_HIP_CHECK(hipStreamWaitEvent(stream, ctx->seg_done, 0));
    ctx->seg_ev_pending = false;
  }
  if (need > ctx->seg_cap) {
    OVN_HIP_CHECK(hipStreamSynchronize(stream));
    if (ctx->seg_dev) (void)hipFree(ctx->seg_dev);
    if (ctx->seg_host) (void)hipHostFree(ctx->seg_host);
    ctx->seg_dev = ctx->seg_host = nullptr;
    ctx->seg_cap = 0;
    const size_t want = need + need / 2;
    OVN_HIP_CHECK(hipMalloc(&ctx->seg_dev, want));
    OVN_HIP_CHECK(hipHostMalloc(&ctx->seg_host, want, hipHostMallocDefault));
    ctx->seg_cap = want;
  }
  OvnCarver hc(ctx->seg_host), dc(ctx->seg_dev);
  const SegTable h(hc, B, qidx != nullptr, n_ridx, n_pseg);
  *dev = SegTable(dc, B, qidx != nullptr, n_ridx, n_pseg);
  memcpy(h.offs, offs, (size_t)(B + 1) * sizeof(int64_t));
  if (qidx) memcpy(h.qidx, qidx, (size_t)B * sizeof(int32_t));
  OVN_HIP_CHECK(hipMemcpyAsync(ctx->seg_dev, ctx->seg_host, staged, hipMemcpyHostToDevice, stream));
  OVN_HIP_CHECK(hipEventRecord(ctx->seg_ev, stream));
  ctx->seg_ev_pending = true;
  return OVN_OK;
}

static int seg_release(ovn_ctx* ctx, hipStream_t stream) {
  OVN_HIP_CHECK(hipEventRecord(ctx->seg_done, stream));
  return OVN_OK;
}

static bool misaligned(const void* p, uintptr_t a) { return (reinterpret_cast<uintptr_t>(p) & (a - 1)) != 0; }

int ovn_heads_segments(ovn_ctx* ctx, const float* feats_pool, const float* spec_pool, const float* dcache_pool,
                       const int32_t* cand_idx, const float* feats_q, const float* spec_q, const int32_t* query_idx,
                       const int64_t* seg_offsets, int64_t B, int64_t n, float* overlap, int32_t* yaw, float* logit, float* corr,
                       void* stream_) {
  OVN_REQUIRE(ctx && ctx->head_set, OVN_ERR_STATE, "ovn_heads_segments: head weights not set");
  int64_t total = 0;
  const char* bad = seg_offsets_error(seg_offsets, B, &total);
  OVN_REQUIRE(bad == nullptr, OVN_ERR_ARG, "ovn_heads_segments: %s", bad);
  OVN_REQUIRE(n == total, OVN_ERR_ARG, "ovn_heads_segments: n = %lld but seg_offsets[B] = %lld", (long long)n, (long long)total);
  OVN_REQUIRE(B == 0 || query_idx != nullptr, OVN_ERR_ARG, "ovn_heads_segments: query_idx is NULL");
  for (int64_t b = 0; b < B; ++b)
    OVN_REQUIRE(query_idx[b] >= 0, OVN_ERR_ARG, "ovn_heads_segments: query_idx[%lld] = %d < 0", (long long)b, query_idx[b]);
  if (n == 0) return OVN_OK;
  OVN_REQUIRE(feats_pool && feats_q && cand_idx && overlap && yaw, OVN_ERR_ARG, "ovn_heads_segments: NULL buffer");
  OVN_REQUIRE((spec_pool == nullptr) == (spec_q == nullptr), OVN_ERR_ARG, "ovn_heads_segments: spec_pool and spec_q go together");
  const int fw = ctx_feat_w(ctx);
  OVN_REQUIRE(spec_pool == nullptr || fw == OVN_FEAT_W, OVN_ERR_ARG,
              "ovn_heads_segments: the spectral correlation head needs 360-column feature volumes (the leg produces %d)", fw);
  OVN_REQUIRE(!misaligned(feats_pool, 4) && !misaligned(feats_q, 4) && !misaligned(cand_idx, 4) && !misaligned(overlap, 4) &&
                  !misaligned(yaw, 4) && !misaligned(logit, 4) && !misaligned(corr, 4) && !misaligned(spec_pool, 4) &&
                  !misaligned(spec_q, 4) && !misaligned(dcache_pool, 16),
              OVN_ERR_ARG, "ovn_heads_segments: misaligned buffer (4 bytes; dcache_pool 16 bytes)");
  OVN_ON_DEVICE(ctx->device);
  hipStream_t stream = (hipStream_t)stream_;
  const bool spectral = spec_pool != nullptr;
  const int corr_mode = spectral ? 2 : 1;
  const bool segmented = ctx->head_mode == 1 && fw == OVN_FEAT_W && ctx->head_s == OVN_S && ctx->head_compact;
  SegTable tab;
  int rc = seg_stage(ctx, seg_offsets, query_idx, B, n, segmented ? n : 0, stream, &tab);
  if (rc) return rc;
  int64_t* offs_dev = tab.offs;
  int32_t *qidx_dev = tab.qidx, *ridx = tab.ridx, *pseg = tab.pseg;
  {
    OvnProfScope ps(ctx, OVN_K_DELTA_PREP, stream);
    rc = ovn_segment_ridx_forward(offs_dev, qidx_dev, (int)B, (int)n, ridx, pseg, stream);
    if (rc) return rc;
  }
  if (!segmented) {
    rc = delta_head_run(ctx, feats_pool, cand_idx, feats_q, ridx, n, overlap, logit, yaw, corr, corr_mode, spec_pool, spec_q, nullptr, stream);
    return rc ? rc : seg_release(ctx, stream);
  }
  const float* dc = spectral ? dcache_pool : nullptr;
  const int64_t* o = seg_offsets;
  auto seg_of = [&](int64_t p) { return (int64_t)(std::upper_bound(o, o + B + 1, p) - o) - 1; };
  for (int64_t p0 = 0; p0 < n;) {
    const int64_t b0 = seg_of(p0);
    int64_t p1 = std::min(n, p0 + ctx->head_chunk);
    if (seg_of(p1 - 1) - b0 + 1 > OVN_SEG_PASS_MAX) p1 = o[b0 + OVN_SEG_PASS_MAX];
    const int64_t np = p1 - p0;
    OvnSegPass sp{pseg + p0, qidx_dev, offs_dev, (int)b0, (int)(seg_of(p1 - 1) - b0 + 1), {}};
    rc = delta_head_run(ctx, feats_pool, cand_idx + p0, feats_q, ridx + p0, np, overlap + p0, logit ? logit + p0 : nullptr, yaw + p0,
                        corr ? corr + (size_t)p0 * fw : nullptr, corr_mode, spec_pool, spec_q, dc, stream, &sp);
    if (rc) return rc;
    p0 = p1;
  }
  return seg_release(ctx, stream);
}

int ovn_top_k_segments(ovn_ctx* ctx, const float* overlap, const int32_t* yaw, const int32_t* ids, const int64_t* seg_offsets,
                       int64_t B, int k, float threshold, int32_t* out, void* stream) {
  OVN_REQUIRE(ctx != nullptr, OVN_ERR_ARG, "ovn_top_k_segments: ctx is NULL");
  OVN_REQUIRE(k >= 1 && k <= OVN_TOP_K_MAX, OVN_ERR_ARG, "ovn_top_k_segments: k must be in 1..OVN_TOP_K_MAX (1024)");
  int64_t n = 0;
  const char* bad = seg_offsets_error(seg_offsets, B, &n);
  OVN_REQUIRE(bad == nullptr, OVN_ERR_ARG, "ovn_top_k_segments: %s", bad);
  if (B == 0) return OVN_OK;
  OVN_REQUIRE(out != nullptr && (n == 0 || overlap != nullptr), OVN_ERR_ARG, "ovn_top_k_segments: NULL buffer");
  OVN_REQUIRE(!misaligned(out, 16), OVN_ERR_ARG, "ovn_top_k_segments: out_dev is not 16-byte aligned");
  OVN_REQUIRE(!misaligned(overlap, 4) && !misaligned(yaw, 4) && !misaligned(ids, 4), OVN_ERR_ARG,
              "ovn_top_k_segments: misaligned buffer");
  OVN_ON_DEVICE(ctx->device);
  SegTable tab;
  int rc = seg_stage(ctx, seg_offsets, nullptr, B, 0, 0, (hipStream_t)stream, &tab);
  if (rc) return rc;
  rc = ovn_top_k_segments_forward(overlap, yaw, ids, tab.offs, (int)B, k, threshold, out, (hipStream_t)stream);
  return rc ? rc : seg_release(ctx, (hipStream_t)stream);
}

int ovn_project(ovn_ctx* ctx, const float* points_dev, const int64_t* offsets_dev, int n_scans,
                int64_t max_points_per_scan, int proj_h, int proj_w, double fov_up_deg, double fov_down_deg,
                double max_range, float* range_dev, float* vertex_dev, float* intensity_dev, int32_t* idx_dev,
                float* normal_dev, float* stacked_dev, int use_depth, int use_normals, int use_intensity, void* stream) {
  OVN_REQUIRE(ctx != nullptr, OVN_ERR_ARG, "ovn_project: ctx is NULL");
  OVN_REQUIRE(n_scans == 0 || (points_dev || max_points_per_scan == 0), OVN_ERR_ARG, "ovn_project: points is NULL");
  OVN_REQUIRE(n_scans == 0 || offsets_dev, OVN_ERR_ARG, "ovn_project: offsets is NULL");
  OVN_ON_DEVICE(ctx->device);
  OvnProfScope ps(ctx, OVN_K_PROJ, (hipStream_t)stream);
  return ovn_project_forward(ctx, points_dev, offsets_dev, n_scans, max_points_per_scan, proj_h, proj_w, fov_up_deg,
                             fov_down_deg, max_range, range_dev, vertex_dev, intensity_dev, idx_dev, normal_dev,
                             stacked_dev, use_depth, use_normals, use_intensity, (hipStream_t)stream);
}

int ovn_project_semantic(ovn_ctx* ctx, const float* points_dev, const int64_t* offsets_dev, int n_scans,
                         int64_t max_points_per_scan, int proj_h, int proj_w, double fov_up_deg, double fov_down_deg,
                         double max_range, const float* probs_dev, int n_classes, float* range_dev, float* vertex_dev,
                         float* intensity_dev, int32_t* idx_dev, float* normal_dev, float* semantic_dev, int32_t* sem_idx_dev,
                         float* stacked_dev, int use_depth, int use_normals, int use_semantic, int use_intensity, void* stream) {
  OVN_REQUIRE(n_classes >= 1 && n_classes <= OVN_SEMANTIC_CLASSES_MAX, OVN_ERR_ARG,
              "ovn_project_semantic: n_classes %d outside 1..%d", n_classes, OVN_SEMANTIC_CLASSES_MAX);
  OVN_REQUIRE(probs_dev || !(semantic_dev || (stacked_dev && use_semantic)), OVN_ERR_ARG,
              "ovn_project_semantic: probabilities requested but probs is NULL");
  OVN_REQUIRE(ctx != nullptr, OVN_ERR_ARG, "ovn_project_semantic: ctx is NULL");
  OVN_REQUIRE(n_scans == 0 || (points_dev || max_points_per_scan == 0), OVN_ERR_ARG, "ovn_project_semantic: points is NULL");
  OVN_REQUIRE(n_scans == 0 || offsets_dev, OVN_ERR_ARG, "ovn_project_semantic: offsets is NULL");
  OVN_ON_DEVICE(ctx->device);
  OvnProfScope ps(ctx, OVN_K_PROJ, (hipStream_t)stream);
  return ovn_project_semantic_forward(ctx, points_dev, offsets_dev, n_scans, max_points_per_scan, proj_h, proj_w, fov_up_deg,
                                      fov_down_deg, max_range, probs_dev, n_classes, range_dev, vertex_dev, intensity_dev, idx_dev,
                                      normal_dev, semantic_dev, sem_idx_dev, stacked_dev, use_depth, use_normals, use_semantic,
                                      use_intensity, (hipStream_t)stream);
}

int ovn_projection_angles(ovn_ctx* ctx, const float* points_dev, int64_t n_points, int proj_h, int proj_w, double fov_up_deg,
                          double fov_down_deg, double max_range, float* yaw_dev, float* pitch_dev, int32_t* pixel_dev,
                          void* stream) {
  OVN_REQUIRE(ctx != nullptr, OVN_ERR_ARG, "ovn_projection_angles: ctx is NULL");
  OVN_REQUIRE(n_points >= 0 && proj_h > 0 && proj_w > 0, OVN_ERR_ARG, "ovn_projection_angles: bad sizes");
  if (n_points == 0) return OVN_OK;
  OVN_REQUIRE(points_dev != nullptr, OVN_ERR_ARG, "ovn_projection_angles: points is NULL");
  OVN_ON_DEVICE(ctx->device);
  return ovn_projection_angles_forward(points_dev, n_points, proj_h, proj_w, fov_up_deg, fov_down_deg, max_range, yaw_dev,
                                       pitch_dev, pixel_dev, (hipStream_t)stream, ctx->proj_trig);
}

int ovn_normals(ovn_ctx* ctx, const float* range_dev, const float* vertex_dev, int n_scans, int proj_h, int proj_w,
                float* normal_dev, void* stream) {
  OVN_REQUIRE(ctx != nullptr, OVN_ERR_ARG, "ovn_normals: ctx is NULL");
  OVN_REQUIRE(n_scans >= 0 && proj_h > 0 && proj_w > 0, OVN_ERR_ARG, "ovn_normals: bad sizes");
  if (n_scans == 0) return OVN_OK;
  OVN_REQUIRE(range_dev && vertex_dev && normal_dev, OVN_ERR_ARG, "ovn_normals: NULL buffer");
  OVN_ON_DEVICE(ctx->device);
  return ovn_normals_forward(range_dev, vertex_dev, n_scans, proj_h, proj_w, normal_dev, (hipStream_t)stream);
}

int ovn_gt_range_images(ovn_ctx* ctx, const float* points_dev, const int64_t* offsets_dev, int n_scans,
                        int64_t max_points_per_scan, const double* ref_poses_dev, const double* inv_cur_pose_dev, int proj_h,
                        int proj_w, double fov_up_deg, double fov_down_deg, double max_range, float* range_dev, void* stream) {
  OVN_REQUIRE(ctx != nullptr, OVN_ERR_ARG, "ovn_gt_range_images: ctx is NULL");
  OVN_REQUIRE(n_scans >= 0 && proj_h > 0 && proj_w > 0 && max_points_per_scan >= 0, OVN_ERR_ARG, "ovn_gt_range_images: bad sizes");
  if (n_scans == 0) return OVN_OK;
  OVN_REQUIRE(offsets_dev && range_dev && (points_dev || max_points_per_scan == 0), OVN_ERR_ARG, "ovn_gt_range_images: NULL buffer");
  OVN_REQUIRE(n_scans <= 65535, OVN_ERR_ARG, "ovn_gt_range_images: at most 65535 scans per call");
  OVN_ON_DEVICE(ctx->device);
  return ovn_gt_range_forward(points_dev, offsets_dev, n_scans, max_points_per_scan, ref_poses_dev, inv_cur_pose_dev, proj_h,
                              proj_w, fov_up_deg, fov_down_deg, max_range, range_dev, (hipStream_t)stream);
}

int ovn_gt_overlap_counts(ovn_ctx* ctx, const float* ref_ranges_dev, const float* cur_range_dev, int n_scans, int proj_h,
                          int proj_w, int32_t* counts_dev, void* stream) {
  OVN_REQUIRE(ctx != nullptr, OVN_ERR_ARG, "ovn_gt_overlap_counts: ctx is NULL");
  OVN_REQUIRE(n_scans >= 0 && proj_h > 0 && proj_w > 0, OVN_ERR_ARG, "ovn_gt_overlap_counts: bad sizes");
  OVN_REQUIRE(cur_range_dev && counts_dev && (ref_ranges_dev || n_scans == 0), OVN_ERR_ARG, "ovn_gt_overlap_counts: NULL buffer");
  OVN_ON_DEVICE(ctx->device);
  return ovn_gt_count_forward(ref_ranges_dev, cur_range_dev, n_scans, proj_h * proj_w, counts_dev, (hipStream_t)stream);
}

int ovn_gt_pair_counts(ovn_ctx* ctx, const float* points_dev, const int64_t* offsets_dev, int n_scans, const double* poses_dev,
                       const double* inv_poses_dev, const float* cur_ranges_dev, const int32_t* frame_idx_dev, int n_frames,
                       const int32_t* ref_idx_dev, int n_refs, int proj_h, int proj_w, double fov_up_deg, double fov_down_deg,
                       double max_range, int32_t* counts_dev, void* stream) {
  OVN_REQUIRE(ctx != nullptr, OVN_ERR_ARG, "ovn_gt_pair_counts: ctx is NULL");
  OVN_REQUIRE(n_scans >= 0 && n_frames >= 0 && n_refs >= 0 && proj_h > 0 && proj_w > 0, OVN_ERR_ARG,
              "ovn_gt_pair_counts: bad sizes");
  OVN_REQUIRE((long long)proj_h * proj_w <= 262144, OVN_ERR_ARG,
              "ovn_gt_pair_counts: %d x %d pixels need %lld bytes of LDS for the two bit planes, 65536 at the most (H*W <= 262144)",
              proj_h, proj_w, 8ll * (((long long)proj_h * proj_w + 31) / 32));
  OVN_REQUIRE((long long)n_frames * n_refs <= 2147483647ll, OVN_ERR_ARG,
              "ovn_gt_pair_counts: %d frames x %d references exceed the grid (2^31 - 1 pairs per call)", n_frames, n_refs);
  if (n_frames == 0 || n_refs == 0) return OVN_OK;
  OVN_REQUIRE(counts_dev != nullptr, OVN_ERR_ARG, "ovn_gt_pair_counts: counts is NULL");
  OVN_REQUIRE(n_scans > 0 && offsets_dev && poses_dev && inv_poses_dev && cur_ranges_dev, OVN_ERR_ARG,
              "ovn_gt_pair_counts: NULL buffer");
  OVN_REQUIRE((frame_idx_dev || n_frames <= n_scans) && (ref_idx_dev || n_refs <= n_scans), OVN_ERR_ARG,
              "ovn_gt_pair_counts: without an index list at most n_scans (%d) frames / references", n_scans);
  int frame_fastest = 1;
  if (const char* e = getenv("OVN_GT_PAIR_ORDER")) frame_fastest = e[0] == 'r' ? 0 : 1;
  OVN_ON_DEVICE(ctx->device);
  return ovn_gt_pair_forward(points_dev, offsets_dev, n_scans, poses_dev, inv_poses_dev, cur_ranges_dev, frame_idx_dev, n_frames,
                             ref_idx_dev, n_refs, proj_h, proj_w, fov_up_deg, fov_down_deg, max_range, frame_fastest, counts_dev,
                             (hipStream_t)stream);
}

int ovn_set_head_precision(ovn_ctx* ctx, int mode) {
  OVN_REQUIRE(ctx != nullptr, OVN_ERR_ARG, "ovn_set_head_precision: ctx is NULL");
  OVN_REQUIRE(mode >= 0 && mode <= 2, OVN_ERR_ARG, "ovn_set_head_precision: mode %d (0 = fp32 MFMA, 1 = f16x3 MFMA, 2 = bf16x3 MFMA)", mode);
  ctx->head_mode = mode;
  return OVN_OK;
}

int ovn_set_head_width_split(ovn_ctx* ctx, int on) {
  OVN_REQUIRE(ctx != nullptr, OVN_ERR_ARG, "ovn_set_head_width_split: ctx is NULL");
  OVN_REQUIRE(on == 0 || on == 1, OVN_ERR_ARG, "ovn_set_head_width_split: %d (0 = exact fp32 at widths other than 360, 1 = f16x3 there)", on);
  ctx->head_width_split = on;
  return OVN_OK;
}

int ovn_get_head_width_split(ovn_ctx* ctx, int* on) {
  OVN_REQUIRE(ctx != nullptr && on != nullptr, OVN_ERR_ARG, "ovn_get_head_width_split: NULL argument");
  *on = ctx->head_width_split;
  return OVN_OK;
}

int ovn_set_corr_normalization(ovn_ctx* ctx, int mode) {
  OVN_REQUIRE(ctx != nullptr, OVN_ERR_ARG, "ovn_set_corr_normalization: ctx is NULL");
  OVN_REQUIRE(mode >= 0 && mode <= 3, OVN_ERR_ARG,
              "ovn_set_corr_normalization: mode %d (0 = none, 1 = euclidean, 2 = scaling, 3 = standardization)", mode);
  ctx->corr_norm = mode;
  return OVN_OK;
}

int ovn_get_corr_normalization(ovn_ctx* ctx, int* mode) {
  OVN_REQUIRE(ctx != nullptr && mode != nullptr, OVN_ERR_ARG, "ovn_get_corr_normalization: NULL argument");
  *mode = ctx->corr_norm;
  return OVN_OK;
}

int ovn_set_head_compaction(ovn_ctx* ctx, int on) {
  OVN_REQUIRE(ctx != nullptr, OVN_ERR_ARG, "ovn_set_head_compaction: ctx is NULL");
  OVN_REQUIRE(on == 0 || on == 1, OVN_ERR_ARG, "ovn_set_head_compaction: %d (0 = walk all 128 channels, 1 = drop the query's dead channels)", on);
  ctx->head_compact = on;
  return OVN_OK;
}

int ovn_set_projection_trig(ovn_ctx* ctx, int mode) {
  OVN_REQUIRE(ctx != nullptr, OVN_ERR_ARG, "ovn_set_projection_trig: ctx is NULL");
  OVN_REQUIRE(mode == 0 || mode == 1, OVN_ERR_ARG, "ovn_set_projection_trig: mode %d (0 = NumPy / SVML float32, 1 = correctly rounded)", mode);
  ctx->proj_trig = mode;
  return OVN_OK;
}

int ovn_set_leg_precision(ovn_ctx* ctx, int mode) {
  OVN_REQUIRE(ctx != nullptr, OVN_ERR_ARG, "ovn_set_leg_precision: ctx is NULL");
  OVN_REQUIRE(mode == 0 || mode == 1, OVN_ERR_ARG, "ovn_set_leg_precision: mode %d (0 = fp32 MFMA, 1 = f16x3 MFMA)", mode);
  if (mode != 0 && ctx->finalized) {
    const int bad = leg_f16x3_unserved(ctx);
    OVN_REQUIRE(bad < 0, OVN_ERR_ARG, "ovn_set_leg_precision: layer %s: fewer than 128 output positions per image in leg precision f16x3",
                ctx->leg[bad < 0 ? 0 : bad].name.c_str());
  }
  ctx->leg_mode = mode;
  return OVN_OK;
}

int ovn_profile_begin(ovn_ctx* ctx) {
  OVN_REQUIRE(ctx != nullptr, OVN_ERR_ARG, "ovn_profile_begin: ctx is NULL");
  for (auto& r : ctx->prof_recs) {
    (void)hipEventDestroy(r.a);
    (void)hipEventDestroy(r.b);
  }
  ctx->prof_recs.clear();
  ctx->prof = true;
  return OVN_OK;
}

int ovn_profile_end(ovn_ctx* ctx, double* ms_by_kind, int64_t* launches_by_kind) {
  OVN_REQUIRE(ctx && ms_by_kind && launches_by_kind, OVN_ERR_ARG, "ovn_profile_end: NULL argument");
  OVN_ON_DEVICE(ctx->device);
  ctx->prof = false;
  for (int k = 0; k < OVN_K_COUNT; ++k) {
    ms_by_kind[k] = 0.0;
    launches_by_kind[k] = 0;
  }
  int rc = OVN_OK;
  for (auto& r : ctx->prof_recs) {
    float ms = 0.f;
    hipError_t e = hipEventSynchronize(r.b);
    if (e == hipSuccess) e = hipEventElapsedTime(&ms, r.a, r.b);
    if (e != hipSuccess) {
      ovn_set_error("ovn_profile_end: %s", hipGetErrorString(e));
      rc = OVN_ERR_HIP;
    } else {
      ms_by_kind[r.kind] += ms;
      launches_by_kind[r.kind] += 1;
    }
    (void)hipEventDestroy(r.a);
    (void)hipEventDestroy(r.b);
  }
  ctx->prof_recs.clear();
  return rc;
}

int ovn_debug_conv(ovn_ctx* ctx, int layer, const float* in_dev, int nb, int h, int w, float* out_dev, void* stream) {
  OVN_REQUIRE(ctx && layer >= 0 && layer < (int)ctx->leg.size(), OVN_ERR_ARG, "ovn_debug_conv: no such leg layer");
  OVN_REQUIRE(in_dev && out_dev && nb >= 0, OVN_ERR_ARG, "ovn_debug_conv: bad buffers");
  OVN_ON_DEVICE(ctx->device);
  int oh = 0, ow = 0;
  if (ctx->leg_mode == 0) return ovn_conv_forward(ctx->leg[layer], in_dev, nb, h, w, out_dev, &oh, &ow, (hipStream_t)stream);
  OVN_REQUIRE(nb <= OVN_LEG_SLICE, OVN_ERR_ARG, "ovn_debug_conv: at most %d images per call", OVN_LEG_SLICE);
  if (!ctx->actmax) OVN_HIP_CHECK(hipMalloc((void**)&ctx->actmax, (size_t)OVN_ACTMAX_SLOTS * OVN_LEG_SLICE * OVN_ACTMAX_STRIDE * sizeof(unsigned)));
  OVN_HIP_CHECK(hipMemsetAsync(ctx->actmax, 0, 2 * (size_t)OVN_LEG_SLICE * OVN_ACTMAX_STRIDE * sizeof(unsigned), (hipStream_t)stream));
  int rc = ovn_absmax_forward(in_dev, nb, (long long)h * w * ctx->leg[layer].cin, ctx->actmax, (hipStream_t)stream);
  if (rc) return rc;
  return ovn_conv_forward_f16x3(ctx->leg[layer], in_dev, nb, h, w, out_dev, &oh, &ow, ctx->actmax, ctx->actmax + (size_t)OVN_LEG_SLICE * OVN_ACTMAX_STRIDE,
                                (hipStream_t)stream);
}

int ovn_debug_head_activations(ovn_ctx* ctx, int64_t n, float* o2_dev, float* o3_dev, void* stream) {
  OVN_REQUIRE(ctx && ctx->dbg_o2 && n >= 0 && n <= ctx->dbg_n, OVN_ERR_STATE,
              "ovn_debug_head_activations: call right after ovn_heads with n <= its (first-chunk) pair count");
  OVN_ON_DEVICE(ctx->device);
  const size_t g = (size_t)ctx->head_g;
  if (o2_dev)
    OVN_HIP_CHECK(hipMemcpyAsync(o2_dev, ctx->dbg_o2, (size_t)n * g * g * OVN_C2_OUT * sizeof(float),
                                 hipMemcpyDeviceToDevice, (hipStream_t)stream));
  if (o3_dev && ctx->dbg_o3)
    OVN_HIP_CHECK(hipMemcpyAsync(o3_dev, ctx->dbg_o3, (size_t)n * (g - 2) * (g - 2) * OVN_C3_OUT * sizeof(float),
                                 hipMemcpyDeviceToDevice, (hipStream_t)stream));
  else if (o3_dev)
    return ovn_c3_dense_forward(ctx, ctx->dbg_o2, ctx->dbg_o2max, (int)n, ctx->dbg_partial, o3_dev, nullptr, nullptr, nullptr, (hipStream_t)stream);
  return OVN_OK;
}

int ovn_head_walk_stats(ovn_ctx* ctx, int32_t* out16_host, void* stream) {
  OVN_REQUIRE(ctx && out16_host, OVN_ERR_ARG, "ovn_head_walk_stats: NULL argument");
  OVN_ON_DEVICE(ctx->device);
  return ovn_delta_walk_stats(ctx, out16_host, (hipStream_t)stream);
}

int64_t ovn_workspace_bytes(ovn_ctx* ctx) { return ctx ? (int64_t)ctx->ws_bytes : 0; }

int ovn_selftest(ovn_ctx* ctx) {
  OVN_REQUIRE(ctx != nullptr, OVN_ERR_ARG, "ovn_selftest: ctx is NULL");
  OVN_ON_DEVICE(ctx->device);
  return ovn_mfma_selftest(nullptr);
}

}
```

overlapnet_amd/csrc/ovn_internal.h:

```cpp
#pragma once

#include <hip/hip_runtime.h>
#include <math.h>
#include <stdint.h>

#include <string>
#include <vector>

#include "../../include/ovn_hip.h"
#include "ovn_scratch.h"

typedef float f32x4 __attribute__((ext_vector_type(4)));

void ovn_set_error(const char* fmt, ...);

#define OVN_HIP_CHECK(expr)                                                                   \
  do {                                                                                        \
    hipError_t _e = (expr);                                                                   \
    if (_e != hipSuccess) {                                                                   \
      ovn_set_error("%s failed: %s (%s:%d)", #expr, hipGetErrorString(_e), __FILE__, __LINE__); \
      return OVN_ERR_HIP;                                                                     \
    }                                                                                         \
  } while (0)

#define OVN_REQUIRE(cond, code, ...)   \
  do {                                 \
    if (!(cond)) {                     \
      ovn_set_error(__VA_ARGS__);      \
      return (code);                   \
    }                                  \
  } while (0)

struct OvnDeviceGuard {
  int prev = -1;
  bool ok = false;
  explicit OvnDeviceGuard(int dev) {
    int cur = -1;
    if (hipGetDevice(&cur) != hipSuccess) return;
    if (cur == dev) {
      ok = true;
      return;
    }
    ok = (hipSetDevice(dev) == hipSuccess);
    if (ok) prev = cur;
  }
  ~OvnDeviceGuard() {
    if (prev >= 0) (void)hipSetDevice(prev);
  }
  OvnDeviceGuard(const OvnDeviceGuard&) = delete;
  OvnDeviceGuard& operator=(const OvnDeviceGuard&) = delete;
};
#define OVN_ON_DEVICE(dev)                                                             \
  OvnDeviceGuard ovn_device_guard_(dev);                                               \
  OVN_REQUIRE(ovn_device_guard_.ok, OVN_ERR_HIP, "cannot select HIP device %d", (int)(dev))

constexpr int OVN_FEAT_W = 360;
constexpr int OVN_FEAT_C = 128;
constexpr int OVN_FEAT_ELEMS = OVN_FEAT_W * OVN_FEAT_C;
constexpr int OVN_S = 15;
constexpr int OVN_G = OVN_FEAT_W / OVN_S;
constexpr int OVN_C1_OUT = 64;
constexpr int OVN_C2_OUT = 128;
constexpr int OVN_C3_OUT = 256;
constexpr int OVN_O3_HW = OVN_G - 2;
constexpr int OVN_DENSE_IN = OVN_O3_HW * OVN_O3_HW * OVN_C3_OUT;
constexpr int OVN_A2_IN_YAW_MAX_PAIRS = 64;
constexpr int OVN_DENSE_PARTIALS = 12;
constexpr int OVN_ACTMAX_SLOTS = 32;
constexpr int OVN_LEG_SLICE = 1024;
constexpr int OVN_ACTMAX_STRIDE = 32;
constexpr int OVN_SPEC_W = 368;
constexpr int OVN_SPEC_ELEMS = OVN_FEAT_C * OVN_SPEC_W;
static_assert(OVN_DELTA_CACHE_ELEMS >= OVN_FEAT_ELEMS + 24 * 128 + 4, "include/ovn_hip.h: OVN_DELTA_CACHE_ELEMS");

__host__ __device__ inline float ovn_pow2_scale_for(float m) {
  if (!(m > 0.0f) || !(m < 3.0e38f)) return 1.0f;
  int e = 0;
  (void)frexpf(m, &e);
  int k = 14 - e;
  k = k > 100 ? 100 : (k < -100 ? -100 : k);
  return ldexpf(1.0f, k);
}

#ifdef __HIPCC__
__device__ __forceinline__ void ovn_fold_absmax_wg(float vmax, unsigned* word, float* red) {
#pragma unroll
  for (int off = 32; off > 0; off >>= 1) vmax = fmaxf(vmax, __shfl_down(vmax, off, 64));
  const int nw = (blockDim.x + 63) >> 6;
  if ((threadIdx.x & 63) == 0) red[threadIdx.x >> 6] = vmax;
  __syncthreads();
  if (threadIdx.x == 0) {
    float m = red[0];
    for (int w = 1; w < nw; ++w) m = fmaxf(m, red[w]);
    const unsigned bits = __float_as_uint(m);
    if (m > 0.f && bits > __hip_atomic_load(word, __ATOMIC_RELAXED, __HIP_MEMORY_SCOPE_AGENT)) atomicMax(word, bits);
  }
}

template <int NWAVES>
__device__ __forceinline__ float ovn_wg_max_all(float m, float* red) {
#pragma unroll
  for (int off = 32; off > 0; off >>= 1) m = fmaxf(m, __shfl_down(m, off, 64));
  if ((threadIdx.x & 63) == 0) red[threadIdx.x >> 6] = m;
  __syncthreads();
  m = red[0];
#pragma unroll
  for (int w = 1; w < NWAVES; ++w) m = fmaxf(m, red[w]);
  return m;
}

typedef _Float16 f16x8 __attribute__((ext_vector_type(8)));
typedef _Float16 f16x4 __attribute__((ext_vector_type(4)));
typedef _Float16 f16x2 __attribute__((ext_vector_type(2)));

__device__ __forceinline__ void ovn_split_f16(float d0, float d1, float s, float one, f16x2& hi, f16x2& lo) {
  const float x0 = d0 * s, x1 = d1 * s;
  hi = __builtin_bit_cast(f16x2, __builtin_amdgcn_cvt_pkrtz(x0, x1));
  lo[0] = (_Float16)__builtin_fmaf(x0, one, -(float)hi[0]);
  lo[1] = (_Float16)__builtin_fmaf(x1, one, -(float)hi[1]);
}
__device__ __forceinline__ void ovn_split_f16(f32x4 d, float s, float one, f16x4& hi, f16x4& lo) {
#pragma unroll
  for (int e = 0; e < 4; e += 2) {
    f16x2 h, l;
    ovn_split_f16(d[e], d[e + 1], s, one, h, l);
    hi[e] = h[0];
    hi[e + 1] = h[1];
    lo[e] = l[0];
    lo[e + 1] = l[1];
  }
}
#endif

constexpr int OVN_NORM_BLK = 24;
constexpr int OVN_NORM_NB = OVN_FEAT_W / OVN_NORM_BLK;
static_assert(OVN_NORM_NB * OVN_NORM_BLK == OVN_FEAT_W, "15 whole blocks tile the 360 columns (the spectral kernels' LDS)");
constexpr int OVN_NORM_NB_MAX = (OVN_FEAT_W_MAX + OVN_NORM_BLK - 1) / OVN_NORM_BLK;

template <int NB, int NCH>
struct OvnNormLds {
  double part[NB][NCH];
  float mn[NB][NCH], mx[NB][NCH];
  double m[NCH], s[NCH];
};

__host__ __device__ inline double ovn_corr_norm_add(int mode) { return mode == 3 ? 1e-5 : 0.0; }

#ifdef __HIPCC__
__device__ __forceinline__ float ovn_corr_norm_apply(float x, double m, double a, double s) {
  return (float)((((double)x - m) + a) * s);
}

__device__ __forceinline__ void ovn_norm_block_stats(const float* __restrict__ p, int n, double& sm, float& lo, float& hi) {
#pragma unroll 8
  for (int i = 0; i < n; ++i) {
    const float v = p[(size_t)i * OVN_FEAT_C];
    sm += (double)v;
    lo = fminf(lo, v);
    hi = fmaxf(hi, v);
  }
}
__device__ __forceinline__ double ovn_norm_block_sumsq(const float* __restrict__ p, int n, double m, double a) {
  double q = 0.0;
#pragma unroll 8
  for (int i = 0; i < n; ++i) {
    const double y = ((double)p[(size_t)i * OVN_FEAT_C] - m) + a;
    q = __builtin_fma(y, y, q);
  }
  return q;
}

template <int NB, int NCH>
__device__ void ovn_corr_norm_affine(const float* __restrict__ X, int W, int mode, OvnNormLds<NB, NCH>& L) {
  const int tid = threadIdx.x, nt = blockDim.x;
  const int nfull = W / OVN_NORM_BLK, tail = W - nfull * OVN_NORM_BLK, nb = nfull + (tail ? 1 : 0);
  for (int t = tid; t < nb * NCH; t += nt) {
    const int c = t % NCH, b = t / NCH;
    const float* p = X + (size_t)(b * OVN_NORM_BLK) * OVN_FEAT_C + c;
    double sm = 0.0;
    float lo = INFINITY, hi = -INFINITY;
    if (b < nfull) ovn_norm_block_stats(p, OVN_NORM_BLK, sm, lo, hi);
    else ovn_norm_block_stats(p, tail, sm, lo, hi);
    L.part[b][c] = sm;
    L.mn[b][c] = lo;
    L.mx[b][c] = hi;
  }
  __syncthreads();
  if (tid < NCH) {
    double sm = 0.0;
    float lo = INFINITY, hi = -INFINITY;
    for (int b = 0; b < nb; ++b) {
      sm += L.part[b][tid];
      lo = fminf(lo, L.mn[b][tid]);
      hi = fmaxf(hi, L.mx[b][tid]);
    }
    if (mode == 2) {
      L.m[tid] = (double)lo;
      L.s[tid] = 1.0 / (((double)hi - (double)lo) + 1e-6);
    } else {
      L.m[tid] = (mode == 3) ? sm / (double)W : 0.0;
      L.s[tid] = 0.0;
    }
  }
  __syncthreads();
  if (mode == 2) return;
  const double a = ovn_corr_norm_add(mode);
  for (int t = tid; t < nb * NCH; t += nt) {
    const int c = t % NCH, b = t / NCH;
    const float* p = X + (size_t)(b * OVN_NORM_BLK) * OVN_FEAT_C + c;
    L.part[b][c] = ovn_norm_block_sumsq(p, b < nfull ? OVN_NORM_BLK : tail, L.m[c], a);
  }
  __syncthreads();
  if (tid < NCH) {
    double q = 0.0;
    for (int b = 0; b < nb; ++b) q += L.part[b][tid];
    L.s[tid] = 1.0 / sqrt(q > 1e-12 ? q : 1e-12);
  }
  __syncthreads();
}
#endif

struct OvnHeadScales {
  float sw1 = 1.f, sw2 = 1.f;
  float sws = 1.f;
  float w1_colsum = 0.f;
  float b1_absmax = 0.f;
};

int ovn_allow_dynamic_lds(const void* kernel, size_t bytes);

struct OvnConvLayer {
  std::string name;
  int kh = 0, kw = 0, cin = 0, cout = 0, sh = 1, sw = 1;
  int relu = 1;
  int out_cols = 0;
  int K = 0;
  int nkc = 0;
  float* wp = nullptr;
  float* bias = nullptr;
  void* wp_h = nullptr;
  float sw_h = 1.f;
  void* wp_h16 = nullptr;
  float* wraw = nullptr;
};

struct ovn_ctx {
  int device = 0;
  int in_h = 0, in_w = 0, in_c = 0;
  std::vector<OvnConvLayer> leg;
  bool finalized = false;
  int feat_w = 0;
  bool head_set = false;
  int head_s = OVN_S;
  int head_g = OVN_G;
  float* w1p = nullptr;
  float* b1 = nullptr;
  OvnConvLayer c2;
  OvnConvLayer c3;
  void* w1p_h = nullptr;
  void* w2p_h = nullptr;
  float* w1raw = nullptr;
  float* w1sum = nullptr;
  float* w1col = nullptr;
  void* wsp_h = nullptr;
  float* w2sum = nullptr;
  void* w1p_b3 = nullptr;
  void* w2p_b3 = nullptr;
  float* w2raw = nullptr;
  float* w3raw = nullptr;
  OvnHeadScales hs;
  int leg_mode = 1;
  int head_compact = 1;
  int proj_trig = 0;
  unsigned* actmax = nullptr;
  int head_mode = 1;
  int head_width_split = 0;
  float* wd = nullptr;
  float* bd = nullptr;
  OvnConvLayer dft;
  double* tw64 = nullptr;
  int corr_norm = 0;
  float* norm_buf = nullptr;
  int64_t norm_buf_n = 0;
  void* comm = nullptr;
  int comm_rank = 0, comm_world = 1;
  int64_t head_chunk = 1024;
  int64_t head_sub = 0;
  int head_streams = 1;
  int head_yaw_side = 0;
  bool aux_ready = false;
  hipStream_t aux[2] = {nullptr, nullptr};
  hipEvent_t ev_fork = nullptr, ev_join[2] = {nullptr, nullptr};
  void* ws = nullptr;
  size_t ws_bytes = 0;
  bool prof = false;
  struct ProfRec {
    hipEvent_t a, b;
    int kind;
  };
  std::vector<ProfRec> prof_recs;
  const float* dbg_o2 = nullptr;
  const float* dbg_o3 = nullptr;
  float* dbg_partial = nullptr;
  const unsigned* dbg_o2max = nullptr;
  int64_t dbg_n = 0;
  unsigned* c3_arrived = nullptr;
  int64_t c3_arrived_n = 0;
  const unsigned* dbg_live = nullptr;
  void* seg_host = nullptr;
  void* seg_dev = nullptr;
  size_t seg_cap = 0;
  hipEvent_t seg_ev = nullptr;
  hipEvent_t seg_done = nullptr;
  bool seg_ev_pending = false;
};

enum { OVN_K_LEG = 0, OVN_K_CORR = 1, OVN_K_DELTA = 2, OVN_K_C3 = 3, OVN_K_DENSE = 4, OVN_K_PROJ = 5, OVN_K_SPECTRUM = 6,
       OVN_K_CORR_SPECTRAL = 7, OVN_K_DELTA_PREP = 8, OVN_K_DELTA_C2 = 9, OVN_K_COUNT = 10 };

struct OvnProfScope {
  ovn_ctx* ctx;
  hipStream_t stream;
  hipEvent_t a = nullptr, b = nullptr;
  int kind;
  OvnProfScope(ovn_ctx* c, int k, hipStream_t s) : ctx(c), stream(s), kind(k) {
    if (ctx->prof && hipEventCreate(&a) == hipSuccess && hipEventCreate(&b) == hipSuccess) (void)hipEventRecord(a, stream);
  }
  ~OvnProfScope() {
    if (ctx->prof && a && b) {
      (void)hipEventRecord(b, stream);
      ctx->prof_recs.push_back({a, b, kind});
    }
  }
};

int ovn_ws_reserve(ovn_ctx* ctx, size_t bytes, hipStream_t stream);
void scratch_overwritten(ovn_ctx* ctx);
template <class L, class... A>
int ovn_ws_layout(ovn_ctx* ctx, hipStream_t stream, L* out, const A&... a) {
  int rc = ovn_ws_reserve(ctx, ovn_scratch_bytes<L>(a...), stream);
  if (rc) return rc;
  OvnCarver c(ctx->ws);
  *out = L(c, a...);
  return OVN_OK;
}

int ovn_conv_prepare(OvnConvLayer* L, const float* kernel_dev, const float* bias_dev, hipStream_t stream);
void ovn_conv_release(OvnConvLayer* L);
int ovn_conv_forward(const OvnConvLayer& L, const float* in, int nb, int h, int w, float* out, int* oh,
                     int* ow, hipStream_t stream);

int ovn_conv_prepare_f16x3(OvnConvLayer* L, const float* kernel_dev, hipStream_t stream);
int ovn_conv_forward_f16x3(const OvnConvLayer& L, const float* in, int nb, int h, int w, float* out, int* oh, int* ow,
                           const unsigned* in_max, unsigned* out_max, hipStream_t stream);
int ovn_absmax_forward(const float* x, int n_scans, long long per_scan, unsigned* out_max, hipStream_t stream);

int ovn_delta_prepare_w1(const float* c1_kernel_dev, float** w1p_out, hipStream_t stream);
struct OvnDeltaF32Scratch {
  float *o2 = nullptr, *o3 = nullptr;
  void* scales = nullptr;
  OvnDeltaF32Scratch() = default;
  OvnDeltaF32Scratch(OvnCarver& c, int64_t n, int G, bool split);
};
size_t ovn_delta_pair_bytes(int G);
int ovn_delta_forward(ovn_ctx* ctx, const float* feats_l, const int32_t* lidx, const float* feats_r, const int32_t* ridx, int n,
                      const OvnDeltaF32Scratch& scratch, float* overlap, float* logit, hipStream_t stream);
int ovn_dense_sigmoid_forward(const ovn_ctx* ctx, const float* o3, int n, long long dense_in, float* overlap, float* logit,
                              hipStream_t stream);

int ovn_delta_prepare_f16x3(ovn_ctx* ctx, const float* c1_kernel_dev, const float* c1_bias_dev, const float* c2_kernel_dev,
                            hipStream_t stream);
struct OvnDeltaSubScratch {
  f32x4* scales = nullptr;
  unsigned *o2max = nullptr, *pl = nullptr, *pr = nullptr;
  float *lin = nullptr, *a2raw = nullptr, *o1raw = nullptr;
  void* desc = nullptr;
  unsigned *qblock = nullptr, *live = nullptr;
  _Float16* w1c = nullptr;
  OvnDeltaSubScratch() = default;
  OvnDeltaSubScratch(OvnCarver& c, int n, bool per_pair_right);
};
struct OvnDeltaSegScratch {
  float* a2raw = nullptr;
  unsigned *qblock = nullptr, *live = nullptr;
  _Float16* w1c = nullptr;
  OvnDeltaSegScratch() = default;
  OvnDeltaSegScratch(OvnCarver& c, int nseg);
};
size_t ovn_delta_f16x3_scratch_bytes(int n, bool per_pair_right);
struct OvnSegPass {
  const int32_t* pseg;
  const int32_t* qidx;
  const int64_t* offs;
  int seg0, nseg;
  OvnDeltaSegScratch state;
};
size_t ovn_delta_f16x3_seg_bytes(int nseg);
int ovn_delta_c12_f16x3_forward(ovn_ctx* ctx, const float* feats_l, const int32_t* lidx, const float* feats_r,
                                const int32_t* ridx, int n, const OvnDeltaSubScratch& scratch, float* o2, hipStream_t stream,
                                int pair0 = 0,
                                const float* dcache_l = nullptr,
                                bool a2_done = false,
                                const struct OvnSegPass* seg = nullptr);
int ovn_delta_c12_bf16x3_forward(ovn_ctx* ctx, const float* feats_l, const int32_t* lidx, const float* feats_r, const int32_t* ridx,
                                 int n, const OvnDeltaSubScratch& scratch, float* o2, hipStream_t stream, int pair0, bool a2_done);
int ovn_delta_cache_forward(ovn_ctx* ctx, const float* feats, int n, float* cache, hipStream_t stream);
int ovn_delta_walk_stats(ovn_ctx* ctx, int32_t* out16, hipStream_t stream);

struct OvnDeltaGenericScratch {
  float *out1 = nullptr, *o2 = nullptr, *o3 = nullptr;
  OvnDeltaGenericScratch() = default;
  OvnDeltaGenericScratch(OvnCarver& c, int64_t n, int W, int G);
};
size_t ovn_delta_generic_pair_bytes(int W, int G);
int ovn_delta_generic_forward(const ovn_ctx* ctx, const float* feats_l, const int32_t* lidx, const float* feats_r,
                              const int32_t* ridx, int n, const OvnDeltaGenericScratch& scratch, float* overlap, float* logit,
                              hipStream_t stream);
int ovn_delta_generic_c1_wide(const ovn_ctx* ctx, int FW, const float* feats_l, const int32_t* lidx, const float* feats_r,
                              const int32_t* ridx, int n, float* out1, hipStream_t stream);

void ovn_head_param_sizes_of(int s, int FW, int64_t* sizes8);
int ovn_delta_head_grad_run(ovn_ctx* ctx, int FW, const float* feats_l, const int32_t* lidx, const float* feats_r, const int32_t* ridx,
                            int64_t n, const float* target, int loss, float scale, float* grad, float* loss_out, float* overlap,
                            float* o2_out, float* o3_out, hipStream_t stream,
                            float* dfeat_l = nullptr, float* dfeat_r = nullptr,
                            bool forward_only = false);

int ovn_delta_data_grad(ovn_ctx* ctx, int FW, const float* feats_l, const int32_t* lidx, const float* feats_r, const int32_t* ridx,
                        const float* dO1, int np, float* dfeat_l, float* dfeat_r, hipStream_t stream);
int ovn_yaw_grad_run(ovn_ctx* ctx, int FW, const float* feats_l, const int32_t* lidx, const float* feats_r, const int32_t* ridx,
                     int64_t n, const float* target, const int32_t* yaw_bin, float yaw_scale, float thr, float* dfeat_l, float* dfeat_r,
                     float* loss_yaw, float* corr, hipStream_t stream);

size_t ovn_leg_grad_part_bytes(const OvnConvLayer& L, int h, int w, int nb);
int ovn_leg_mask_forward(const float* dy, const float* y, float* out, long long n, hipStream_t stream);
int ovn_leg_grad_round(const double* acc, float* out, long long n, hipStream_t stream);
int ovn_leg_layer_backward(const OvnConvLayer& L, const float* x, const float* dym, int nb, int h, int w, float* dx, const float* mask,
                           double* acc_kernel, double* acc_bias, double* part, hipStream_t stream);

size_t ovn_delta_w_split_pair_bytes();
int ovn_delta_w_split_c12_forward(ovn_ctx* ctx, const float* feats_l, const int32_t* lidx, const float* feats_r, const int32_t* ridx,
                                  int n, void* scales, float* o2, hipStream_t stream);

int ovn_corr_forward(const float* feats_l, const int32_t* lidx, const float* feats_r, const int32_t* ridx, int n, int W,
                     int32_t* yaw, float* corr, hipStream_t stream, int norm_mode);

int ovn_spectral_prepare(ovn_ctx* ctx, hipStream_t stream);
int ovn_spectrum_forward(ovn_ctx* ctx, const float* feats, int n, float* spectra, hipStream_t stream);
bool ovn_conv_strip_own_scale(const OvnConvLayer& L, int h, int w);
bool ovn_conv_strip_matches(const OvnConvLayer& L, int h, int w);
int ovn_conv_strip_try(const OvnConvLayer& L, const float* in, int nb, int h, int w, float* out, const unsigned* in_max,
                       unsigned* out_max, hipStream_t stream);

bool ovn_leg_front_matches(const ovn_ctx* ctx, size_t first, int h, int w);
int ovn_leg_front_forward(const ovn_ctx* ctx, size_t first, const float* in, int nb, int h, int w, float* out, int* oh_out, int* ow_out,
                          unsigned* out_max, hipStream_t stream);

bool ovn_leg_tail_matches(const ovn_ctx* ctx, size_t first, int h, int w);
int ovn_leg_tail_forward(const ovn_ctx* ctx, size_t first, const float* in, int nb, int w, float* out, hipStream_t stream);

int ovn_c3_dense_forward(const ovn_ctx* ctx, const float* o2, const unsigned* o2max, int n, float* partial, float* o3,
                         unsigned* arrived, float* overlap, float* logit, hipStream_t stream);

int ovn_gt_range_forward(const float* points, const int64_t* offsets, int n_scans, long long max_points, const double* ref_poses,
                         const double* inv_cur_pose, int H, int W, double fov_up_deg, double fov_down_deg, double max_range,
                         float* range_out, hipStream_t stream);
int ovn_gt_count_forward(const float* ref_ranges, const float* cur_range, int n, int npix, int32_t* counts, hipStream_t stream);
int ovn_gt_pair_forward(const float* points, const int64_t* offsets, int n_scans, const double* poses, const double* inv_poses,
                        const float* cur_ranges, const int32_t* frame_idx, int n_frames, const int32_t* ref_idx, int n_refs, int H,
                        int W, double fov_up_deg, double fov_down_deg, double max_range, int frame_fastest, int32_t* counts,
                        hipStream_t stream);
int ovn_best_match_forward(const float* overlap, const int32_t* yaw, const int32_t* ids, int n, float threshold,
                           int index_offset, int32_t* out, hipStream_t stream);
int ovn_top_k_forward(const float* overlap, const int32_t* yaw, const int32_t* ids, int n, int k, float threshold,
                      int index_offset, int32_t* out, hipStream_t stream);
int ovn_top_k_segments_forward(const float* overlap, const int32_t* yaw, const int32_t* ids, const int64_t* offs_dev, int B, int k,
                               float threshold, int32_t* out, hipStream_t stream);
int ovn_segment_ridx_forward(const int64_t* offs_dev, const int32_t* qidx_dev, int B, int n, int32_t* ridx, int32_t* pseg,
                             hipStream_t stream);
int ovn_icp_register_forward(const float* vertex, const float* normal, const float* range, int n_scans, int H, int W,
                             double fov_up_deg, double fov_down_deg, double max_range, const int32_t* src_idx, const int32_t* tgt_idx,
                             int n_pairs, const double* init_pose, int iterations, double max_dist, double cos_min, double huber,
                             int min_inliers, double* pose, double* stats, double* system, hipStream_t stream);
int ovn_corr_spectral_forward(ovn_ctx* ctx, const float* spec_l, const int32_t* lidx, const float* spec_r,
                              const int32_t* ridx, int n, int32_t* yaw, float* corr, hipStream_t stream,
                              const float* a2_feats_r = nullptr, float* a2raw = nullptr);

int ovn_project_forward(ovn_ctx* ctx, const float* points, const int64_t* offsets, int n_scans,
                        int64_t max_points, int H, int W, double fov_up_deg, double fov_down_deg,
                        double max_range, float* range, float* vertex, float* intensity, int32_t* idx,
                        float* normal, float* stacked, int use_depth, int use_normals, int use_intensity,
                        hipStream_t stream);

int ovn_project_semantic_forward(ovn_ctx* ctx, const float* points, const int64_t* offsets, int n_scans, int64_t max_points, int H,
                                 int W, double fov_up_deg, double fov_down_deg, double max_range, const float* probs, int n_classes,
                                 float* range, float* vertex, float* intensity, int32_t* idx, float* normal, float* semantic,
                                 int32_t* sem_idx, float* stacked, int use_depth, int use_normals, int use_semantic, int use_intensity,
                                 hipStream_t stream);
int ovn_projection_angles_forward(const float* points, int64_t n, int H, int W, double fov_up_deg, double fov_down_deg,
                                  double max_range, float* yaw, float* pitch, int32_t* pixel, hipStream_t stream, int trig = 0);
int ovn_normals_forward(const float* range, const float* vertex, int n_scans, int H, int W, float* normal,
                        hipStream_t stream);

int ovn_mfma_selftest(hipStream_t stream);
```

Baseline: 235,700.

## Split conv3+dense into six pixel-tile bands with fragment-ordered dense weights

Replaces the three row bands of the fused conv3+Dense kernel with six bands of up to six 16-pixel M-tiles, cut in raster pixel order. It uses 4-wave workgroups tuned for two workgroups per CU, and the number of N-tiles per wave is a template parameter (1, 2 or 4) picked from the batch size. Dense weights are reordered once, at setup, into MFMA fragment order so the epilogue can read them contiguously. The change is meant to improve occupancy and load balance, and to shrink the LDS patch per workgroup. In exchange there are more partials per pair (96 instead of 12), which need a separate partial buffer and a longer finishing reduction, and some input halo is reloaded across bands.

```diff
diff --git a/overlapnet_amd/csrc/c3_bands.h b/overlapnet_amd/csrc/c3_bands.h
--- /dev/null
+++ b/overlapnet_amd/csrc/c3_bands.h
@@ -0,0 +1,45 @@
+#pragma once
+
+constexpr int C3B_G = 24;
+constexpr int C3B_OW = 22;
+constexpr int C3B_CI = 128;
+constexpr int C3B_CO = 256;
+constexpr int C3B_NPIX = C3B_OW * C3B_OW;
+constexpr int C3B_TILES = (C3B_NPIX + 15) / 16;
+constexpr int C3B_NBAND = 6;
+constexpr int C3B_MAX_MT = 6;
+constexpr int C3B_NT = C3B_CO / 16;
+
+constexpr int c3b_first_tile(int b) { return 5 * b; }
+constexpr int c3b_tiles(int b) { return b == C3B_NBAND - 1 ? C3B_TILES - c3b_first_tile(b) : 5; }
+constexpr int c3b_first_pixel(int b) { return 16 * c3b_first_tile(b); }
+constexpr int c3b_pixels(int b) { return b == C3B_NBAND - 1 ? C3B_NPIX - c3b_first_pixel(b) : 16 * c3b_tiles(b); }
+constexpr int c3b_raster(int p) { return (p / C3B_OW) * C3B_G + p % C3B_OW; }
+constexpr int C3B_TAP_MAX = 2 * C3B_G + 2;
+constexpr int c3b_origin(int b) { return c3b_raster(c3b_first_pixel(b)); }
+constexpr int c3b_span(int b) { return c3b_raster(c3b_first_pixel(b) + c3b_pixels(b) - 1) + C3B_TAP_MAX + 1 - c3b_origin(b); }
+constexpr int c3b_max_span() {
+  int m = 0;
+  for (int b = 0; b < C3B_NBAND; ++b) m = c3b_span(b) > m ? c3b_span(b) : m;
+  return m;
+}
+constexpr int C3B_MAX_SPAN = c3b_max_span();
+
+constexpr int C3B_NPL = C3B_CI / 8;
+constexpr int C3B_PLANE = C3B_MAX_SPAN * 8 + 8;
+constexpr int C3B_LDS_BYTES = 2 * C3B_NPL * C3B_PLANE * 2;
+constexpr int C3B_PATCH_LOADS = (C3B_MAX_SPAN * C3B_CI / 4 + 255) / 256;
+
+constexpr int C3B_WDF_ELEMS = C3B_NBAND * C3B_NT * C3B_MAX_MT * 64 * 4;
+constexpr int c3b_wdf_index(int band, int nt, int mt, int lane, int r) {
+  return (((band * C3B_NT + nt) * C3B_MAX_MT + mt) * 64 + lane) * 4 + r;
+}
+constexpr int c3b_wdf_source(int band, int nt, int mt, int lane, int r) {
+  const int p = 16 * mt + 4 * (lane >> 4) + r;
+  return (mt < c3b_tiles(band) && p < c3b_pixels(band)) ? (c3b_first_pixel(band) + p) * C3B_CO + 16 * nt + (lane & 15) : -1;
+}
+
+static_assert(c3b_first_tile(C3B_NBAND - 1) + c3b_tiles(C3B_NBAND - 1) == C3B_TILES && c3b_tiles(C3B_NBAND - 1) == C3B_MAX_MT, "bands");
+static_assert(c3b_origin(C3B_NBAND - 1) + c3b_span(C3B_NBAND - 1) == C3B_G * C3B_G, "the last band ends with the input");
+static_assert(C3B_PATCH_LOADS <= 18, "patch loads per thread");
+static_assert(C3B_LDS_BYTES <= 80 * 1024 && 2 * C3B_LDS_BYTES <= 160 * 1024, "two workgroups share a CU's 160 KB of LDS");
diff --git a/overlapnet_amd/csrc/c3_dense.hip b/overlapnet_amd/csrc/c3_dense.hip
--- a/overlapnet_amd/csrc/c3_dense.hip
+++ b/overlapnet_amd/csrc/c3_dense.hip
@@ -1,7 +1,5 @@
 #include "ovn_internal.h"
-
-typedef _Float16 f16x8 __attribute__((ext_vector_type(8)));
-typedef _Float16 f16x4 __attribute__((ext_vector_type(4)));
+#include "c3_bands.h"
 
 namespace {
 
@@ -12,75 +10,75 @@
   static __device__ __forceinline__ f32x4 mfma(v8 a, v8 b, f32x4 c) { return __builtin_amdgcn_mfma_f32_16x16x32_f16(a, b, c, 0, 0, 0); }
 };
 
-constexpr int G = OVN_G;
-constexpr int OW = OVN_O3_HW;
-constexpr int CI = OVN_C2_OUT;
-constexpr int CO = OVN_C3_OUT;
-constexpr int NBAND = 3;
-constexpr int MAX_ROWS = 8;
-constexpr int MAX_MT = (MAX_ROWS * OW + 15) / 16;
-constexpr int IN_PIX_MAX = (MAX_ROWS + 2) * G;
-constexpr int PLANE = IN_PIX_MAX * 8 + 8;
-constexpr int NPL = CI / 8;
-constexpr size_t LDS_BYTES = 2 * (size_t)NPL * PLANE * sizeof(_Float16) + 64;
-constexpr int NW = 8;
-
-__device__ __forceinline__ int band_start(int b) { return b == 0 ? 0 : (b == 1 ? 8 : 15); }
-__device__ __forceinline__ int band_rows(int b) { return b == 0 ? 8 : 7; }
-
-constexpr int MT_SPLIT = 6;
-template <class A, int NWV, int MSPLIT>
-__global__ __launch_bounds__(64 * NWV) void c3_dense_kernel(const float* __restrict__ o2, const typename A::elem* __restrict__ wp,
-                                                           const float* __restrict__ b3, const float* __restrict__ wd,
-                                                           const unsigned* __restrict__ o2max, float sw3,
-                                                           float* __restrict__ partial, float* __restrict__ o3,
-                                                           unsigned* __restrict__ arrived, const float* __restrict__ bd,
-                                                           float* __restrict__ overlap, float* __restrict__ logit) {
+static_assert(C3B_G == OVN_G && C3B_OW == OVN_O3_HW && C3B_CI == OVN_C2_OUT && C3B_CO == OVN_C3_OUT, "c3_bands.h describes this network");
+static_assert(OVN_DENSE_PARTIALS == C3B_NBAND * C3B_NT, "one Dense partial per (band, n-tile)");
+constexpr int G = C3B_G;
+constexpr int CI = C3B_CI;
+constexpr int CO = C3B_CO;
+constexpr int NBAND = C3B_NBAND;
+constexpr int MAX_MT = C3B_MAX_MT;
+constexpr int PLANE = C3B_PLANE;
+constexpr int NPL = C3B_NPL;
+constexpr size_t LDS_BYTES = C3B_LDS_BYTES;
+constexpr int NWV = 4;
+
+template <class Load>
+__device__ __forceinline__ float dense_finish_sum(Load q, const float* __restrict__ bd) {
+  float z = 0.f;
+#pragma unroll
+  for (int b = 0; b < NBAND; ++b) {
+    float zb = q(C3B_NT * b);
+#pragma unroll
+    for (int nt = 1; nt < C3B_NT; ++nt) zb += q(C3B_NT * b + nt);
+    z = b == 0 ? zb : z + zb;
+  }
+  return z + bd[0];
+}
+
+template <class A, int NTW>
+__global__ __launch_bounds__(64 * NWV, 2) void c3_dense_kernel(const float* __restrict__ o2, const typename A::elem* __restrict__ wp,
+                                                              const float* __restrict__ b3, const float* __restrict__ wdf,
+                                                              const unsigned* __restrict__ o2max, float sw3,
+                                                              float* __restrict__ partial, float* __restrict__ o3,
+                                                              unsigned* __restrict__ arrived, const float* __restrict__ bd,
+                                                              float* __restrict__ overlap, float* __restrict__ logit) {
   typedef typename A::elem elem_t;
   typedef typename A::v8 v8_t;
   typedef typename A::v4 v4_t;
   extern __shared__ __attribute__((aligned(16))) unsigned char smem[];
   elem_t* ih = reinterpret_cast<elem_t*>(smem);
   elem_t* il = ih + NPL * PLANE;
-  float* red = reinterpret_cast<float*>(il + NPL * PLANE);
-
-  constexpr int HALVES = NW / NWV;
-  constexpr int MTW = MSPLIT == 1 ? MAX_MT : MT_SPLIT;
-  const int sub = blockIdx.x % (HALVES * MSPLIT);
-  const int unit = blockIdx.x / (HALVES * MSPLIT), half = sub % HALVES, mh = sub / HALVES;
-  const int mt0 = MT_SPLIT * mh;
+
+  constexpr int CG = C3B_NT / (NWV * NTW);
+  const int cg = blockIdx.x % CG;
+  const int unit = blockIdx.x / CG;
   const int pair = unit / NBAND;
   const int band = unit - pair * NBAND;
-  const int r0 = band_start(band);
-  const int nrows = band_rows(band);
-  const int npix = nrows * OW;
-  const int nmt = (npix + 15) >> 4;
+  const int p0 = c3b_first_pixel(band);
+  const int npix = c3b_pixels(band);
+  const bool six = band == NBAND - 1;
+  const int org = c3b_origin(band);
   const int tid = threadIdx.x;
   const int lane = tid & 63;
-  const int wave_l = tid >> 6;
-  const int wave = wave_l + NWV * half;
+  const int nt0 = (cg * NWV + (tid >> 6)) * NTW;
   const int lrow = lane & 15;
   const int g = lane >> 4;
 
-  const elem_t* wsrc = wp + ((size_t)(2 * wave) * 2) * 512 + lane * 8;
-  v8_t bq[3][4];
+  const elem_t* wsrc = wp + ((size_t)nt0 * 2) * 512 + lane * 8;
+  v8_t bq[3][2 * NTW];
 #define C3_LOAD_B(DST, KC)                                                                  \
   {                                                                                         \
-    const elem_t* q = wsrc + (size_t)(KC) * (16 * 2 * 512);                                 \
-    DST[0] = *reinterpret_cast<const v8_t*>(q);                                           \
-    DST[1] = *reinterpret_cast<const v8_t*>(q + 512);                                     \
-    DST[2] = *reinterpret_cast<const v8_t*>(q + 1024);                                    \
-    DST[3] = *reinterpret_cast<const v8_t*>(q + 1536);                                    \
+    const elem_t* q = wsrc + (size_t)(KC) * (C3B_NT * 2 * 512);                             \
+    _Pragma("unroll") for (int j = 0; j < 2 * NTW; ++j) DST[j] = *reinterpret_cast<const v8_t*>(q + 512 * j); \
   }
   C3_LOAD_B(bq[0], 0)
   C3_LOAD_B(bq[1], 1)
   const float s2 = ovn_pow2_scale_for(__uint_as_float(o2max[pair]));
   const float inv = 1.0f / (s2 * sw3);
   {
-    const float* src = o2 + ((long long)pair * G + r0) * G * CI;
-    const int n4 = (nrows + 2) * G * CI / 4;
-    constexpr int PER_THREAD = (MAX_ROWS + 2) * G * CI / 4 / (64 * NWV);
-    static_assert(PER_THREAD * 64 * NWV == (MAX_ROWS + 2) * G * CI / 4, "patch does not divide over the threads");
+    const float* src = o2 + ((long long)pair * (G * G) + org) * CI;
+    const int n4 = c3b_span(band) * (CI / 4);
+    constexpr int PER_THREAD = C3B_PATCH_LOADS;
     f32x4 v[PER_THREAD];
 #pragma unroll
     for (int k = 0; k < PER_THREAD; ++k) {
@@ -107,68 +105,64 @@
     }
   }
 
-  int abase[MTW];
-#pragma unroll
-  for (int mt = 0; mt < MTW; ++mt) {
-    int p = 16 * (mt0 + mt) + lrow;
+  int abase[MAX_MT];
+#pragma unroll
+  for (int mt = 0; mt < MAX_MT; ++mt) {
+    int p = 16 * mt + lrow;
     if (p >= npix) p = npix - 1;
-    const int oy = p / OW;
-    const int ox = p - oy * OW;
-    abase[mt] = g * PLANE + (oy * G + ox) * 8;
-  }
-
-  f32x4 acc[MTW][2];
-#pragma unroll
-  for (int mt = 0; mt < MTW; ++mt) {
-    acc[mt][0] = (f32x4){0.f, 0.f, 0.f, 0.f};
-    acc[mt][1] = (f32x4){0.f, 0.f, 0.f, 0.f};
-  }
-
+    abase[mt] = g * PLANE + (c3b_raster(p0 + p) - org) * 8;
+  }
+
+  f32x4 acc[MAX_MT][NTW];
+#pragma unroll
+  for (int mt = 0; mt < MAX_MT; ++mt)
+#pragma unroll
+    for (int nt = 0; nt < NTW; ++nt) acc[mt][nt] = (f32x4){0.f, 0.f, 0.f, 0.f};
+
+#define C3_MFMA1(M0, A0H, A0L, SRC)                                                               \
+  _Pragma("unroll") for (int nt = 0; nt < NTW; ++nt) acc[M0][nt] = A::mfma(A0H, SRC[2 * nt], acc[M0][nt]);     \
+  _Pragma("unroll") for (int nt = 0; nt < NTW; ++nt) acc[M0][nt] = A::mfma(A0L, SRC[2 * nt], acc[M0][nt]);     \
+  _Pragma("unroll") for (int nt = 0; nt < NTW; ++nt) acc[M0][nt] = A::mfma(A0H, SRC[2 * nt + 1], acc[M0][nt]);
 #define C3_MFMA2(M0, M1, A0H, A0L, A1H, A1L, SRC)                                                  \
-  acc[M0][0] = A::mfma(A0H, SRC[0], acc[M0][0]);          \
-  acc[M0][1] = A::mfma(A0H, SRC[2], acc[M0][1]);          \
-  acc[M1][0] = A::mfma(A1H, SRC[0], acc[M1][0]);          \
-  acc[M1][1] = A::mfma(A1H, SRC[2], acc[M1][1]);          \
-  acc[M0][0] = A::mfma(A0L, SRC[0], acc[M0][0]);          \
-  acc[M0][1] = A::mfma(A0L, SRC[2], acc[M0][1]);          \
-  acc[M1][0] = A::mfma(A1L, SRC[0], acc[M1][0]);          \
-  acc[M1][1] = A::mfma(A1L, SRC[2], acc[M1][1]);          \
-  acc[M0][0] = A::mfma(A0H, SRC[1], acc[M0][0]);          \
-  acc[M0][1] = A::mfma(A0H, SRC[3], acc[M0][1]);          \
-  acc[M1][0] = A::mfma(A1H, SRC[1], acc[M1][0]);          \
-  acc[M1][1] = A::mfma(A1H, SRC[3], acc[M1][1]);
+  _Pragma("unroll") for (int nt = 0; nt < NTW; ++nt) {                                             \
+    acc[M0][nt] = A::mfma(A0H, SRC[2 * nt], acc[M0][nt]);                                          \
+    acc[M1][nt] = A::mfma(A1H, SRC[2 * nt], acc[M1][nt]);                                          \
+  }                                                                                                \
+  _Pragma("unroll") for (int nt = 0; nt < NTW; ++nt) {                                             \
+    acc[M0][nt] = A::mfma(A0L, SRC[2 * nt], acc[M0][nt]);                                          \
+    acc[M1][nt] = A::mfma(A1L, SRC[2 * nt], acc[M1][nt]);                                          \
+  }                                                                                                \
+  _Pragma("unroll") for (int nt = 0; nt < NTW; ++nt) {                                             \
+    acc[M0][nt] = A::mfma(A0H, SRC[2 * nt + 1], acc[M0][nt]);                                      \
+    acc[M1][nt] = A::mfma(A1H, SRC[2 * nt + 1], acc[M1][nt]);                                      \
+  }
 #define C3_READ_A(BUF, SLOT, MT)                                                            \
-  fh[BUF][SLOT] = *reinterpret_cast<const v8_t*>(ih + abase[MT] + toff);                  \
+  fh[BUF][SLOT] = *reinterpret_cast<const v8_t*>(ih + abase[MT] + toff);                    \
   fl[BUF][SLOT] = *reinterpret_cast<const v8_t*>(il + abase[MT] + toff);
 #define C3_STEP(SRC, KC)                                                                    \
   {                                                                                         \
     const int tap = (KC) >> 2;                                                              \
     const int ky = tap / 3;                                                                 \
     const int toff = (ky * G + (tap - 3 * ky)) * 8 + 4 * PLANE * ((KC) & 3);                \
-    v8_t fh[2][2], fl[2][2];                                                              \
+    v8_t fh[2][2], fl[2][2];                                                                \
     C3_READ_A(0, 0, 0)                                                                      \
     C3_READ_A(0, 1, 1)                                                                      \
-    _Pragma("unroll") for (int q = 0; q < MTW / 2; ++q) {                                \
-      const int cb = q & 1, nb = cb ^ 1;                                                    \
-      if (q + 1 < MTW / 2) {                                                             \
-        C3_READ_A(nb, 0, 2 * q + 2)                                                         \
-        C3_READ_A(nb, 1, 2 * q + 3)                                                         \
-      } else if (MTW % 2 == 1 && nmt == MAX_MT) {                                                           \
-        C3_READ_A(nb, 0, MTW - 1)                                                        \
-      }                                                                                     \
-      __builtin_amdgcn_sched_barrier(0);   \
-      C3_MFMA2(2 * q, 2 * q + 1, fh[cb][0], fl[cb][0], fh[cb][1], fl[cb][1], SRC)           \
-      __builtin_amdgcn_sched_barrier(0);                                                    \
+    C3_READ_A(1, 0, 2)                                                                      \
+    C3_READ_A(1, 1, 3)                                                                      \
+    __builtin_amdgcn_sched_barrier(0);   \
+    C3_MFMA2(0, 1, fh[0][0], fl[0][0], fh[0][1], fl[0][1], SRC)                             \
+    __builtin_amdgcn_sched_barrier(0);                                                      \
+    C3_READ_A(0, 0, 4)                                                                      \
+    if (six) { C3_READ_A(0, 1, 5) }                                                         \
+    __builtin_amdgcn_sched_barrier(0);                                                      \
+    C3_MFMA2(2, 3, fh[1][0], fl[1][0], fh[1][1], fl[1][1], SRC)                             \
+    __builtin_amdgcn_sched_barrier(0);                                                      \
+    if (six) {                                                                              \
+      C3_MFMA2(4, 5, fh[0][0], fl[0][0], fh[0][1], fl[0][1], SRC)                           \
+    } else {                                                                                \
+      C3_MFMA1(4, fh[0][0], fl[0][0], SRC)                                                  \
     }                                                                                       \
-    if (MTW % 2 == 1 && nmt == MAX_MT) {                               \
-      const v8_t ah = fh[(MTW / 2) & 1][0], al = fl[(MTW / 2) & 1][0];              \
-      acc[MTW - 1][0] = A::mfma(ah, SRC[0], acc[MTW - 1][0]); \
-      acc[MTW - 1][1] = A::mfma(ah, SRC[2], acc[MTW - 1][1]); \
-      acc[MTW - 1][0] = A::mfma(al, SRC[0], acc[MTW - 1][0]); \
-      acc[MTW - 1][1] = A::mfma(al, SRC[2], acc[MTW - 1][1]); \
-      acc[MTW - 1][0] = A::mfma(ah, SRC[1], acc[MTW - 1][0]); \
-      acc[MTW - 1][1] = A::mfma(ah, SRC[3], acc[MTW - 1][1]); \
-    }                                                                                       \
+    __builtin_amdgcn_sched_barrier(0);                                                      \
   }
   __syncthreads();
 #pragma unroll 1
@@ -182,66 +176,45 @@
   }
 #undef C3_LOAD_B
 #undef C3_STEP
+#undef C3_MFMA1
 #undef C3_MFMA2
 #undef C3_READ_A
 
-  float s[2] = {0.f, 0.f};
-#pragma unroll
-  for (int nt = 0; nt < 2; ++nt) {
-    const int n = 32 * wave + 16 * nt + lrow;
+#pragma unroll
+  for (int nt = 0; nt < NTW; ++nt) {
+    const int n = 16 * (nt0 + nt) + lrow;
     const float bv = b3[n];
-#pragma unroll
-    for (int mt = 0; mt < MTW; ++mt) {
-#pragma unroll
-      for (int r = 0; r < 4; ++r) {
-        const int p = 16 * (mt0 + mt) + 4 * g + r;
-        if (p < npix) {
-          const float v = fmaxf(fmaf(acc[mt][nt][r], inv, bv), 0.0f);
-          const long long fi = (long long)(r0 * OW + p) * CO + n;
-          s[(MSPLIT == 1 && mt >= MT_SPLIT) ? 1 : 0] += v * wd[fi];
-          if (o3) o3[(long long)pair * OVN_DENSE_IN + fi] = v;
+    const float* wq = wdf + c3b_wdf_index(band, nt0 + nt, 0, lane, 0);
+    float s = 0.f;
+#pragma unroll
+    for (int mt = 0; mt < MAX_MT; ++mt) {
+      if (mt < MAX_MT - 1 || six) {
+        const f32x4 w = *reinterpret_cast<const f32x4*>(wq + c3b_wdf_index(0, 0, mt, 0, 0));
+#pragma unroll
+        for (int r = 0; r < 4; ++r) {
+          const int p = 16 * mt + 4 * g + r;
+          if (mt < MAX_MT - 1 || p < npix) {
+            const float v = fmaxf(fmaf(acc[mt][nt][r], inv, bv), 0.0f);
+            s += v * w[r];
+            if (o3) o3[(long long)pair * OVN_DENSE_IN + (long long)(p0 + p) * CO + n] = v;
+          }
         }
       }
     }
-  }
-#pragma unroll
-  for (int off = 32; off > 0; off >>= 1) {
-    s[0] += __shfl_down(s[0], off, 64);
-    if (MSPLIT == 1) s[1] += __shfl_down(s[1], off, 64);
-  }
-  if (lane == 0) {
-    red[wave_l] = s[0];
-    if (MSPLIT == 1) red[NW + wave_l] = s[1];
-  }
-  __syncthreads();
-  if (tid == 0) {
-    float* dst = partial + ((size_t)pair * NBAND + band) * 4;
-    if (NWV == NW) {
-      dst[0] = (red[0] + red[1]) + (red[2] + red[3]);
-      dst[1] = (red[NW + 0] + red[NW + 1]) + (red[NW + 2] + red[NW + 3]);
-      dst[2] = (red[4] + red[5]) + (red[6] + red[7]);
-      dst[3] = (red[NW + 4] + red[NW + 5]) + (red[NW + 6] + red[NW + 7]);
-    } else {
-      dst[2 * half + mh] = (red[0] + red[1]) + (red[2] + red[3]);
-    }
-    if (overlap != nullptr) {
-      constexpr unsigned PARTS = NBAND * HALVES * MSPLIT;
-      __threadfence();
+#pragma unroll
+    for (int off = 32; off > 0; off >>= 1) s += __shfl_down(s, off, 64);
+    if (lane == 0) partial[((size_t)pair * NBAND + band) * C3B_NT + nt0 + nt] = s;
+  }
+  if (overlap != nullptr) {
+    __threadfence();
+    __syncthreads();
+    if (tid == 0) {
+      constexpr unsigned PARTS = NBAND * CG;
       const unsigned prev = atomicAdd(arrived + pair, 1u);
       if (prev == PARTS - 1) {
         __threadfence();
         const float* q = partial + (size_t)pair * OVN_DENSE_PARTIALS;
-        float z = 0.f;
-#pragma unroll
-        for (int b = 0; b < NBAND; ++b) {
-          const float q0 = __hip_atomic_load(q + 4 * b, __ATOMIC_RELAXED, __HIP_MEMORY_SCOPE_AGENT);
-          const float q1 = __hip_atomic_load(q + 4 * b + 1, __ATOMIC_RELAXED, __HIP_MEMORY_SCOPE_AGENT);
-          const float q2 = __hip_atomic_load(q + 4 * b + 2, __ATOMIC_RELAXED, __HIP_MEMORY_SCOPE_AGENT);
-          const float q3 = __hip_atomic_load(q + 4 * b + 3, __ATOMIC_RELAXED, __HIP_MEMORY_SCOPE_AGENT);
-          const float zb = (q0 + q1) + (q2 + q3);
-          z = b == 0 ? zb : z + zb;
-        }
-        z += bd[0];
+        const float z = dense_finish_sum([q](int i) { return __hip_atomic_load(q + i, __ATOMIC_RELAXED, __HIP_MEMORY_SCOPE_AGENT); }, bd);
         if (logit) logit[pair] = z;
         overlap[pair] = 1.0f / (1.0f + expf(-z));
         __hip_atomic_store(arrived + pair, 0u, __ATOMIC_RELAXED, __HIP_MEMORY_SCOPE_AGENT);
@@ -255,39 +228,57 @@
   const int p = blockIdx.x * 256 + threadIdx.x;
   if (p >= n) return;
   const float* q = partial + (size_t)p * OVN_DENSE_PARTIALS;
-  float z = 0.f;
-#pragma unroll
-  for (int b = 0; b < NBAND; ++b) {
-    const float zb = (q[4 * b] + q[4 * b + 1]) + (q[4 * b + 2] + q[4 * b + 3]);
-    z = b == 0 ? zb : z + zb;
-  }
-  z += bd[0];
+  const float z = dense_finish_sum([q](int i) { return q[i]; }, bd);
   if (logit) logit[p] = z;
   overlap[p] = 1.0f / (1.0f + expf(-z));
 }
 
+__global__ __launch_bounds__(256) void dense_fragment_order_kernel(const float* __restrict__ wd, float* __restrict__ wdf) {
+  const int i = blockIdx.x * 256 + threadIdx.x;
+  if (i >= C3B_WDF_ELEMS) return;
+  const int r = i & 3, lane = (i >> 2) & 63;
+  const int t = i >> 8;
+  const int mt = t % C3B_MAX_MT, nt = (t / C3B_MAX_MT) % C3B_NT, band = t / (C3B_MAX_MT * C3B_NT);
+  const int src = c3b_wdf_source(band, nt, mt, lane, r);
+  wdf[i] = src >= 0 ? wd[src] : 0.0f;
+}
+
+template <int NTW>
+int launch_c3_dense(const ovn_ctx* ctx, const float* o2, const unsigned* o2max, int n, float* partial, float* o3, unsigned* arrived,
+                    float* overlap, float* logit, hipStream_t stream) {
+  int rc = ovn_allow_dynamic_lds(reinterpret_cast<const void*>(c3_dense_kernel<ArithF16, NTW>), LDS_BYTES);
+  if (rc) return rc;
+  hipLaunchKernelGGL((c3_dense_kernel<ArithF16, NTW>), dim3(NBAND * (C3B_NT / (NWV * NTW)) * n), dim3(64 * NWV), LDS_BYTES, stream, o2,
+                     reinterpret_cast<const _Float16*>(ctx->c3.wp_h), ctx->c3.bias, ctx->wd_frag, o2max, ctx->c3.sw_h, partial, o3, arrived,
+                     ctx->bd, overlap, logit);
+  return OVN_OK;
+}
+
+}
+
+int ovn_c3_dense_prepare_wd(const float* wd, float** wdf_out, hipStream_t stream) {
+  OVN_HIP_CHECK(hipMalloc((void**)wdf_out, (size_t)C3B_WDF_ELEMS * sizeof(float)));
+  hipLaunchKernelGGL(dense_fragment_order_kernel, dim3((C3B_WDF_ELEMS + 255) / 256), dim3(256), 0, stream, wd, *wdf_out);
+  OVN_HIP_CHECK(hipGetLastError());
+  return OVN_OK;
 }
 
 int ovn_c3_dense_forward(const ovn_ctx* ctx, const float* o2, const unsigned* o2max, int n, float* partial, float* o3,
                          unsigned* arrived, float* overlap, float* logit, hipStream_t stream) {
   OVN_REQUIRE(o2max != nullptr, OVN_ERR_ARG, "ovn_c3_dense_forward: the per-pair maxima of o2 are required");
   OVN_REQUIRE(overlap == nullptr || arrived != nullptr, OVN_ERR_ARG, "ovn_c3_dense_forward: arrival counters missing");
+  OVN_REQUIRE(ctx->wd_frag != nullptr, OVN_ERR_STATE, "ovn_c3_dense_forward: no fragment-order Dense kernel registered");
   int rc;
-  if (n <= 21) {
-    rc = ovn_allow_dynamic_lds(reinterpret_cast<const void*>(c3_dense_kernel<ArithF16, 4, 2>), LDS_BYTES);
-    if (rc) return rc;
-    hipLaunchKernelGGL((c3_dense_kernel<ArithF16, 4, 2>), dim3(4 * NBAND * n), dim3(64 * 4), LDS_BYTES, stream, o2,
-                       reinterpret_cast<const _Float16*>(ctx->c3.wp_h), ctx->c3.bias, ctx->wd, o2max, ctx->c3.sw_h, partial, o3, arrived,
-                       ctx->bd, overlap, logit);
-  } else {
-    rc = ovn_allow_dynamic_lds(reinterpret_cast<const void*>(c3_dense_kernel<ArithF16, NW, 1>), LDS_BYTES);
-    if (rc) return rc;
-    hipLaunchKernelGGL((c3_dense_kernel<ArithF16, NW, 1>), dim3(NBAND * n), dim3(64 * NW), LDS_BYTES, stream, o2,
-                       reinterpret_cast<const _Float16*>(ctx->c3.wp_h), ctx->c3.bias, ctx->wd, o2max, ctx->c3.sw_h, partial, o3,
-                       (unsigned*)nullptr, ctx->bd, (float*)nullptr, (float*)nullptr);
-    if (overlap != nullptr)
+  if (n <= 4)
+    rc = launch_c3_dense<1>(ctx, o2, o2max, n, partial, o3, arrived, overlap, logit, stream);
+  else if (n <= 21)
+    rc = launch_c3_dense<2>(ctx, o2, o2max, n, partial, o3, arrived, overlap, logit, stream);
+  else {
+    rc = launch_c3_dense<4>(ctx, o2, o2max, n, partial, o3, nullptr, nullptr, nullptr, stream);
+    if (rc == OVN_OK && overlap != nullptr)
       hipLaunchKernelGGL(dense_finish_kernel, dim3((n + 255) / 256), dim3(256), 0, stream, partial, ctx->bd, n, overlap, logit);
   }
+  if (rc) return rc;
   OVN_HIP_CHECK(hipGetLastError());
   return OVN_OK;
 }
diff --git a/overlapnet_amd/csrc/ovn_api.hip b/overlapnet_amd/csrc/ovn_api.hip
--- a/overlapnet_amd/csrc/ovn_api.hip
+++ b/overlapnet_amd/csrc/ovn_api.hip
@@ -116,6 +116,7 @@
   if (ctx->w1p) (void)hipFree(ctx->w1p);
   if (ctx->b1) (void)hipFree(ctx->b1);
   if (ctx->wd) (void)hipFree(ctx->wd);
+  if (ctx->wd_frag) (void)hipFree(ctx->wd_frag);
   if (ctx->bd) (void)hipFree(ctx->bd);
   if (ctx->w1p_h) (void)hipFree(ctx->w1p_h);
   if (ctx->w2p_h) (void)hipFree(ctx->w2p_h);
@@ -132,6 +133,7 @@
   if (ctx->norm_buf) (void)hipFree(ctx->norm_buf);
   if (ctx->actmax) (void)hipFree(ctx->actmax);
   if (ctx->c3_arrived) (void)hipFree(ctx->c3_arrived);
+  if (ctx->c3_partial) (void)hipFree(ctx->c3_partial);
   if (ctx->seg_dev) (void)hipFree(ctx->seg_dev);
   if (ctx->seg_host) (void)hipHostFree(ctx->seg_host);
   if (ctx->seg_ev) (void)hipEventDestroy(ctx->seg_ev);
@@ -215,6 +217,7 @@
     if (ctx->w1p) (void)hipFree(ctx->w1p);
     if (ctx->b1) (void)hipFree(ctx->b1);
     if (ctx->wd) (void)hipFree(ctx->wd);
+    if (ctx->wd_frag) (void)hipFree(ctx->wd_frag);
     if (ctx->bd) (void)hipFree(ctx->bd);
     if (ctx->w1p_h) (void)hipFree(ctx->w1p_h);
     if (ctx->w2p_h) (void)hipFree(ctx->w2p_h);
@@ -230,7 +233,7 @@
     ctx->w3raw = nullptr;
     ctx->w1p_h = ctx->w2p_h = ctx->wsp_h = ctx->w1p_b3 = ctx->w2p_b3 = nullptr;
     ctx->w1raw = ctx->w1sum = ctx->w1col = ctx->w2sum = ctx->w2raw = nullptr;
-    ctx->w1p = ctx->b1 = ctx->wd = ctx->bd = nullptr;
+    ctx->w1p = ctx->b1 = ctx->wd = ctx->wd_frag = ctx->bd = nullptr;
     ctx->head_set = false;
   }
   ctx->head_g = ctx_feat_w(ctx) / ctx->head_s;
@@ -291,6 +294,10 @@
   OVN_HIP_CHECK(hipMalloc((void**)&ctx->bd, sizeof(float)));
   OVN_HIP_CHECK(hipMemcpyAsync(ctx->wd, dk, dense_in * sizeof(float), hipMemcpyDeviceToDevice, stream));
   OVN_HIP_CHECK(hipMemcpyAsync(ctx->bd, db, sizeof(float), hipMemcpyDeviceToDevice, stream));
+  if (!general && hg == OVN_G) {
+    rc = ovn_c3_dense_prepare_wd(ctx->wd, &ctx->wd_frag, stream);
+    if (rc) return rc;
+  }
   OVN_HIP_CHECK(hipStreamSynchronize(stream));
   ctx->head_set = true;
   return OVN_OK;
@@ -716,7 +723,7 @@
   HeadScratch() = default;
   HeadScratch(OvnCarver& c, int64_t cmax, bool fused, int64_t sub_pairs, int nsub, bool per_pair_right, int nseg) {
     o2 = c.take<float>((size_t)cmax * OVN_G * OVN_G * OVN_C2_OUT);
-    o3 = c.take<float>((size_t)cmax * (fused ? OVN_DENSE_PARTIALS : OVN_DENSE_IN));
+    o3 = c.take<float>((size_t)cmax * (fused ? 12 : OVN_DENSE_IN));
     sub_bytes = ovn_delta_f16x3_scratch_bytes((int)sub_pairs, per_pair_right);
     sub = c.take<char>(sub_bytes * nsub);
     if (nseg) seg = OvnDeltaSegScratch(c, nseg);
@@ -750,9 +757,12 @@
   if (fused && ctx->c3_arrived_n < chunk) {
     OVN_HIP_CHECK(hipStreamSynchronize(stream));
     if (ctx->c3_arrived) (void)hipFree(ctx->c3_arrived);
+    if (ctx->c3_partial) (void)hipFree(ctx->c3_partial);
     ctx->c3_arrived = nullptr;
+    ctx->c3_partial = nullptr;
     ctx->c3_arrived_n = 0;
     OVN_HIP_CHECK(hipMalloc((void**)&ctx->c3_arrived, (size_t)chunk * sizeof(unsigned)));
+    OVN_HIP_CHECK(hipMalloc((void**)&ctx->c3_partial, (size_t)chunk * OVN_DENSE_PARTIALS * sizeof(float)));
     OVN_HIP_CHECK(hipMemsetAsync(ctx->c3_arrived, 0, (size_t)chunk * sizeof(unsigned), stream));
     ctx->c3_arrived_n = chunk;
   }
@@ -760,7 +770,7 @@
   ctx->dbg_o2max = nullptr;
   ctx->dbg_o2 = o2;
   ctx->dbg_o3 = fused ? nullptr : o3;
-  ctx->dbg_partial = fused ? o3 : nullptr;
+  ctx->dbg_partial = fused ? ctx->c3_partial : nullptr;
   ctx->dbg_n = sub < cmax ? sub : cmax;
 
   OvnFork fk(ctx, stream);
@@ -802,7 +812,7 @@
       const OvnDeltaSubScratch ds = hs.sub_chunk(j, np, ridx != nullptr);
       if (fused) {
         unsigned* o2max = ds.o2max;
-        float* part = o3 + (size_t)q0 * OVN_DENSE_PARTIALS;
+        float* part = ctx->c3_partial + (size_t)q0 * OVN_DENSE_PARTIALS;
         OvnSegPass sp{};
         if (seg) {
           sp = *seg;
diff --git a/overlapnet_amd/csrc/ovn_internal.h b/overlapnet_amd/csrc/ovn_internal.h
--- a/overlapnet_amd/csrc/ovn_internal.h
+++ b/overlapnet_amd/csrc/ovn_internal.h
@@ -65,7 +65,7 @@
 constexpr int OVN_O3_HW = OVN_G - 2;
 constexpr int OVN_DENSE_IN = OVN_O3_HW * OVN_O3_HW * OVN_C3_OUT;
 constexpr int OVN_A2_IN_YAW_MAX_PAIRS = 64;
-constexpr int OVN_DENSE_PARTIALS = 12;
+constexpr int OVN_DENSE_PARTIALS = 96;
 constexpr int OVN_ACTMAX_SLOTS = 32;
 constexpr int OVN_LEG_SLICE = 1024;
 constexpr int OVN_ACTMAX_STRIDE = 32;
@@ -276,6 +276,7 @@
   int head_mode = 1;
   int head_width_split = 0;
   float* wd = nullptr;
+  float* wd_frag = nullptr;
   float* bd = nullptr;
   OvnConvLayer dft;
   double* tw64 = nullptr;
@@ -306,6 +307,7 @@
   int64_t dbg_n = 0;
   unsigned* c3_arrived = nullptr;
   int64_t c3_arrived_n = 0;
+  float* c3_partial = nullptr;
   const unsigned* dbg_live = nullptr;
   void* seg_host = nullptr;
   void* seg_dev = nullptr;
@@ -459,6 +461,7 @@
 bool ovn_leg_tail_matches(const ovn_ctx* ctx, size_t first, int h, int w);
 int ovn_leg_tail_forward(const ovn_ctx* ctx, size_t first, const float* in, int nb, int w, float* out, hipStream_t stream);
 
+int ovn_c3_dense_prepare_wd(const float* wd, float** wdf_out, hipStream_t stream);
 int ovn_c3_dense_forward(const ovn_ctx* ctx, const float* o2, const unsigned* o2max, int n, float* partial, float* o3,
                          unsigned* arrived, float* overlap, float* logit, hipStream_t stream);
 
```

After: 233,100 (median of 2 runs). No clear change (-1.1%).
